# xxayt/MGSV

Hardware: AMD Instinct MI355X
Metric: video-music pairs/s fwd+bwd at B=64 (full training step); sub-objects: retrieval sim-matrix GB/s, eval forward pairs/s (higher is better)
Workload: dtype bf16; 1 GPU; BASELINE.json configs[2]: B=64/GPU, T_v=30, T_a=512, D=512, train mode (dropout on), f32 master weights + Adam, f32 gradient accumulation; global_batch=64, launch=tape

## Files before the change

include/made_hip.h:

```cpp
#ifndef MADE_HIP_H
#define MADE_HIP_H

#include <stdint.h>

#ifdef __cplusplus
extern "C" {
#endif

#define MADE_ABI_VERSION 8

enum MadeDtype { MADE_F32 = 0, MADE_BF16 = 1 };

enum MadeAct {
    MADE_ACT_NONE = 0,
    MADE_ACT_RELU = 1,
    MADE_ACT_GELU = 2,
    MADE_ACT_QUICKGELU = 3,
    MADE_ACT_SIGMOID = 4
};

enum MadeGate {
    MADE_GATE_NONE = 0,
    MADE_GATE_RELU_OUT = 1,
    MADE_GATE_GELU_Z = 2,
// ... 54 lines not shown
    int32_t use_a2;
    int32_t _pad;
} MadeLinearSeg;

typedef struct MadeLinearArgs {
    const void*  A;  int32_t a_dtype; int32_t w_dtype;
    int64_t      lda;
    const void*  A2; int64_t lda2; int64_t a2_row_mod;
    int32_t      a2_replace;
    int32_t      drop_col_div;
    const float* a_row_mask;
    const void*  W;  int64_t ldw;
    const float* bias;
    int64_t      M, N, K;
    int64_t      batch, a_z_stride, w_z_stride;
    int32_t      act; int32_t r_dtype;
    const void*  R;  int64_t ldr; int64_t r_row_mod;
    const float* out_row_mask;
    const float* tile_skip_mask;
    int32_t      nseg; int32_t split_k;
    float*       split_ws;
    MadeLinearSeg seg[4];
    const void*  G;  int32_t g_dtype; int32_t gate;
    int64_t      ldg; float gate_scale; int32_t z_dtype;
    void*        Zout; int64_t ldz;
    MadeDropout  drop; int64_t drop_ld;
    const int32_t* row_index; const int32_t* n_rows;
    const float* bias_row_scale; int64_t bias_z_stride;
} MadeLinearArgs;

int made_linear(const MadeLinearArgs* args, void* stream);

enum MadeLinearVariant {
    MADE_LINEAR_GENERAL_F32 = 0,
    MADE_LINEAR_GENERAL_F32IN = 1,
    MADE_LINEAR_GENERAL_BF16 = 2,
    MADE_LINEAR_TINY = 3,
    MADE_LINEAR_SKINNY = 4,
    MADE_LINEAR_GLDS3 = 5,
    MADE_LINEAR_GLDS64 = 6,
    MADE_LINEAR_GLDS128 = 7,
    MADE_LINEAR_BIG256 = 8,
    MADE_LINEAR_TINY16 = 9,
    MADE_LINEAR_BIG128 = 10,
    MADE_LINEAR_GLDS64_F32 = 11,
    MADE_LINEAR_GLDS128_F32 = 12
};
int made_linear_variant(const MadeLinearArgs* args);

typedef struct MadeDecStageArgs {
    const void*  Zin; int64_t ldz;
    const float* ln_g; const float* ln_b;
    const float* ln2_g; const float* ln2_b; void* x2_out; int64_t ldx2;
    const void*  add; int64_t add_row_mod;
    void*        x_out; int64_t ldx;
    const void*  W; int64_t ldw; const float* bias;
    const void*  R; int64_t ldr;
    void*        out; int64_t ldo;
    int32_t      out_dtype; int32_t act; int32_t res_from_x; float eps;
    int64_t      M, N, K;
    int32_t      zin_dtype; int32_t drop_col_div;
    void*        a_out; int64_t lda_out;
    MadeDropout  drop; int64_t drop_ld;
} MadeDecStageArgs;
int made_dec_stage(const MadeDecStageArgs* args, void* stream);

typedef struct MadeDecStageBwdArgs {
    const void* xa; const float* gamma_a; int64_t ldxa;
    const void* xb; const float* gamma_b; int64_t ldxb;
    const void* dy; int64_t lddy;
    const void* add; int64_t ldadd;
    void* dx_out; int64_t lddx;
    void* a_out; int64_t lda_out;
    float *dgamma_a, *dbeta_a, *dgamma_b, *dbeta_b;
    MadeDropout drop_a; int64_t drop_a_ld;
    const void* W; int64_t ldw;
    const void* G; int64_t ldg; float gate_scale; float eps;
    MadeDropout drop_o; int64_t drop_o_ld; int32_t drop_o_col_div; int32_t _pad;
    const void* R; int64_t ldr;
    void* out; int64_t ldo;
    int64_t M, N, K;
} MadeDecStageBwdArgs;
int made_dec_stage_bwd(const MadeDecStageBwdArgs* args, void* stream);

typedef struct MadeFinishArgs {
    const float* ws; int64_t split_k, M, N;
    const float* bias; int32_t act; int32_t r_dtype;
    const void*  R; int64_t ldr; int64_t r_row_mod;
    void* out; int32_t out_dtype; int32_t _pad0; int64_t ldo;
    const float* ln1_g; const float* ln1_b; void* ln1_out; int32_t ln1_dtype; int32_t _pad1; int64_t ln1_ld;
    const float* ln2_g; const float* ln2_b; void* ln2_out; int32_t ln2_dtype; int32_t _pad2; int64_t ln2_ld;
    float eps; int32_t _pad3;
} MadeFinishArgs;

int made_splitk_finish(const MadeFinishArgs* args, void* stream);

typedef struct MadeAttnArgs {
    const void* Q; const void* K; const void* V; void* O;
    int32_t dtype; int32_t hd;
    int64_t B, H, Lq, Lk;
    int64_t q_bs, ldq, k_bs, ldk, v_bs, ldv, o_bs, ldo;
    const float* key_mask; const float* q_mask;
    float scale; int32_t _pad;
    const float* q_skip_mask;
    float*      lse;
    MadeDropout drop;
    const int32_t* batch_order;
    uint32_t* keep_bits;
    int64_t ld_bits;
} MadeAttnArgs;

int made_attention(const MadeAttnArgs* args, void* stream);

typedef struct MadeWideAttnArgs {
    const void* Q; const void* K; const void* Kadd; const void* V; void* O;
    const float* key_mask;
    int32_t dtype; int32_t o_dtype;
    int64_t B, NQ1, NQ2, L, D;
    int64_t q_bs, q_s1, q_s2, k_bs, ldk, kadd_bs, ldkadd, v_bs, ldv, o_bs, o_s1, o_s2;
    float scale; int32_t _pad;
    int64_t n_split;
    float*  part_o;
    float*  part_ml;
    MadeDropout drop;
    float*  sum_out;
    float*  lse_out;
} MadeWideAttnArgs;

int made_attention_wide(const MadeWideAttnArgs* args, void* stream);

typedef struct MadeWideAttnBwdArgs {
    const void *Q, *dO, *O, *K, *V;
    const float* key_mask;
    const float *lse, *ssum;
    const float* extra;
    const void* dattc; int64_t ld_dattc; const float* vbias; int64_t hd;
    void *Pd, *dS; int64_t p_bs, ld_p;
    void* dQ; int64_t dq_bs, ld_dq;
    int64_t B, NQ, L, D;
    int64_t q_bs, ld_q, do_bs, ld_do, o_bs, ld_o, k_bs, ldk, v_bs, ldv;
    float scale; int32_t _pad;
    int64_t n_split; float* part_dq;
    MadeDropout drop;
} MadeWideAttnBwdArgs;
int made_attention_wide_bwd(const MadeWideAttnBwdArgs* args, void* stream);

#define MADE_WIDE_PLAN_HEAD 4
#define MADE_WIDE_PLAN_SAMPLE 4
#define MADE_WIDE_PLAN_SLOT 16
#define MADE_WIDE_PLAN_SLOT_BITS 8
MADE_HOST_DEVICE static inline int64_t made_wide_plan_words(int64_t B, int64_t n_slots) {
    return MADE_WIDE_PLAN_HEAD + MADE_WIDE_PLAN_SAMPLE * B + MADE_WIDE_PLAN_SLOT * n_slots;
}
MADE_HOST_DEVICE static inline int32_t made_wide_slice_count(const int32_t* tiles, int32_t stride, int32_t B, int32_t c, int32_t max_slices) {
    int32_t total = 0;
    for (int32_t b = 0; b < B; ++b) {
        const int32_t t = tiles[b * stride];
        const int32_t n = t > c ? (t + c - 1) / c : 1;
        if (n > max_slices) return -1;
        total += n;
    }
    return total;
}
MADE_HOST_DEVICE static inline int32_t made_wide_slice_cap(const int32_t* tiles, int32_t stride, int32_t B, int32_t n_slots, int32_t max_slices) {
    int32_t tmax = 1;
    for (int32_t b = 0; b < B; ++b) tmax = tiles[b * stride] > tmax ? tiles[b * stride] : tmax;
// ... 459 lines not shown
```

mgsv_amd/_lib.py:

```python
from __future__ import annotations

import ctypes as C
import os

_HERE = os.path.dirname(os.path.abspath(__file__))


def variant_env(name: str, default: str = "") -> str:
    if os.environ.get("MADE_DEBUG_VARIANTS", "0") in ("", "0"):
        return default
    return os.environ.get(name, default)


LIB_PATH = os.environ.get("MADE_LIB_PATH") or os.path.join(_HERE, "libmade_hip.so")
ABI_VERSION = 8

F32, BF16 = 0, 1
ACT_NONE, ACT_RELU, ACT_GELU, ACT_QUICKGELU, ACT_SIGMOID = 0, 1, 2, 3, 4
GATE_NONE, GATE_RELU_OUT, GATE_GELU_Z, GATE_QUICKGELU_Z, GATE_SIGMOID_OUT = 0, 1, 2, 3, 4

vp, i64, i32, f32 = C.c_void_p, C.c_int64, C.c_int32, C.c_float

WIDE_PLAN_HEAD, WIDE_PLAN_SAMPLE, WIDE_PLAN_SLOT, WIDE_PLAN_SLOT_BITS = 4, 4, 16, 8


def wide_plan_words(B: int, n_slots: int) -> int:
    return WIDE_PLAN_HEAD + WIDE_PLAN_SAMPLE * B + WIDE_PLAN_SLOT * n_slots


class MadeDropout(C.Structure):
    _fields_ = [("seed", C.c_uint64), ("site", C.c_uint32), ("p", f32), ("seed_device", vp)]


class MadeLinearSeg(C.Structure):
    _fields_ = [("col_begin", i64), ("out", vp), ("out_dtype", i32), ("transposed", i32), ("ldo", i64),
                ("rows_per_batch", i64), ("out_batch_stride", i64), ("out_z_stride", i64),
                ("use_a2", i32), ("_pad", i32)]


class MadeLinearArgs(C.Structure):
    _fields_ = [("A", vp), ("a_dtype", i32), ("w_dtype", i32), ("lda", i64),
                ("A2", vp), ("lda2", i64), ("a2_row_mod", i64),
                ("a2_replace", i32), ("drop_col_div", i32),
                ("a_row_mask", vp),
                ("W", vp), ("ldw", i64),
                ("bias", vp),
                ("M", i64), ("N", i64), ("K", i64),
                ("batch", i64), ("a_z_stride", i64), ("w_z_stride", i64),
                ("act", i32), ("r_dtype", i32),
                ("R", vp), ("ldr", i64), ("r_row_mod", i64),
                ("out_row_mask", vp),
                ("tile_skip_mask", vp),
                ("nseg", i32), ("split_k", i32),
                ("split_ws", vp),
                ("seg", MadeLinearSeg * 4),
                ("G", vp), ("g_dtype", i32), ("gate", i32), ("ldg", i64), ("gate_scale", f32), ("z_dtype", i32),
                ("Zout", vp), ("ldz", i64), ("drop", MadeDropout), ("drop_ld", i64), ("row_index", vp), ("n_rows", vp),
                ("bias_row_scale", vp), ("bias_z_stride", i64)]


class MadeFinishArgs(C.Structure):
    _fields_ = [("ws", vp), ("split_k", i64), ("M", i64), ("N", i64),
                ("bias", vp), ("act", i32), ("r_dtype", i32),
                ("R", vp), ("ldr", i64), ("r_row_mod", i64),
                ("out", vp), ("out_dtype", i32), ("_pad0", i32), ("ldo", i64),
                ("ln1_g", vp), ("ln1_b", vp), ("ln1_out", vp), ("ln1_dtype", i32), ("_pad1", i32), ("ln1_ld", i64),
                ("ln2_g", vp), ("ln2_b", vp), ("ln2_out", vp), ("ln2_dtype", i32), ("_pad2", i32), ("ln2_ld", i64),
                ("eps", f32), ("_pad3", i32)]


class MadeDecStageArgs(C.Structure):
    _fields_ = [("Zin", vp), ("ldz", i64), ("ln_g", vp), ("ln_b", vp),
                ("ln2_g", vp), ("ln2_b", vp), ("x2_out", vp), ("ldx2", i64),
                ("add", vp), ("add_row_mod", i64), ("x_out", vp), ("ldx", i64),
                ("W", vp), ("ldw", i64), ("bias", vp), ("R", vp), ("ldr", i64), ("out", vp), ("ldo", i64),
                ("out_dtype", i32), ("act", i32), ("res_from_x", i32), ("eps", f32),
                ("M", i64), ("N", i64), ("K", i64),
                ("zin_dtype", i32), ("drop_col_div", i32), ("a_out", vp), ("lda_out", i64), ("drop", MadeDropout), ("drop_ld", i64)]


class MadeDecStageBwdArgs(C.Structure):
    _fields_ = [("xa", vp), ("gamma_a", vp), ("ldxa", i64), ("xb", vp), ("gamma_b", vp), ("ldxb", i64), ("dy", vp), ("lddy", i64),
                ("add", vp), ("ldadd", i64), ("dx_out", vp), ("lddx", i64), ("a_out", vp), ("lda_out", i64),
                ("dgamma_a", vp), ("dbeta_a", vp), ("dgamma_b", vp), ("dbeta_b", vp), ("drop_a", MadeDropout), ("drop_a_ld", i64),
                ("W", vp), ("ldw", i64), ("G", vp), ("ldg", i64), ("gate_scale", f32), ("eps", f32),
                ("drop_o", MadeDropout), ("drop_o_ld", i64), ("drop_o_col_div", i32), ("_pad", i32),
                ("R", vp), ("ldr", i64), ("out", vp), ("ldo", i64), ("M", i64), ("N", i64), ("K", i64)]


class MadeAttnArgs(C.Structure):
    _fields_ = [("Q", vp), ("K", vp), ("V", vp), ("O", vp),
                ("dtype", i32), ("hd", i32),
                ("B", i64), ("H", i64), ("Lq", i64), ("Lk", i64),
                ("q_bs", i64), ("ldq", i64), ("k_bs", i64), ("ldk", i64),
                ("v_bs", i64), ("ldv", i64), ("o_bs", i64), ("ldo", i64),
                ("key_mask", vp), ("q_mask", vp),
                ("scale", f32), ("_pad", i32),
                ("q_skip_mask", vp),
                ("lse", vp), ("drop", MadeDropout), ("batch_order", vp), ("keep_bits", vp), ("ld_bits", i64)]


class MadeAttnBwdArgs(C.Structure):
    _fields_ = [("Q", vp), ("K", vp), ("V", vp), ("O", vp), ("dO", vp), ("dQ", vp), ("dK", vp), ("dV", vp),
                ("lse", vp), ("delta", vp), ("dtype", i32), ("hd", i32),
                ("B", i64), ("H", i64), ("Lq", i64), ("Lk", i64),
                ("q_bs", i64), ("ldq", i64), ("k_bs", i64), ("ldk", i64), ("v_bs", i64), ("ldv", i64), ("o_bs", i64), ("ldo", i64),
                ("do_bs", i64), ("lddo", i64), ("dq_bs", i64), ("lddq", i64), ("dk_bs", i64), ("lddk", i64), ("dv_bs", i64), ("lddv", i64),
                ("key_mask", vp), ("q_skip_mask", vp), ("scale", f32), ("_pad", i32), ("drop", MadeDropout),
                ("batch_order", vp), ("keep_bits", vp), ("ld_bits", i64)]


class MadeXpoolFusedArgs(C.Structure):
    _fields_ = [("Q", vp), ("ldq", i64), ("K", vp), ("U", vp), ("k_bs", i64), ("ldk", i64), ("u_bs", i64), ("ldu", i64),
                ("key_mask", vp), ("ln2_g", vp), ("ln2_b", vp), ("Wl", vp), ("ldw", i64), ("bl", vp), ("ln3_g", vp), ("ln3_b", vp),
                ("vn", vp), ("ldvn", i64), ("sims", vp), ("ld_sims", i64),
                ("Nv", i64), ("Nm", i64), ("S", i64), ("D", i64), ("scale", f32), ("eps", f32), ("ws", vp), ("prepare_ws", i32), ("_pad", i32)]


class MadeXpoolAttnArgs(C.Structure):
    _fields_ = [("Q", vp), ("ldq", i64), ("K", vp), ("U", vp), ("k_bs", i64), ("ldk", i64), ("u_bs", i64), ("ldu", i64),
                ("key_mask", vp), ("out", vp), ("ldo", i64), ("Nv", i64), ("Nm", i64), ("S", i64), ("D", i64),
                ("scale", f32), ("eps", f32), ("normalize", i32), ("_pad", i32), ("ws", vp)]


class MadeXpoolSimsArgs(C.Structure):
    _fields_ = [("Q", vp), ("ldq", i64), ("K", vp), ("UU", vp), ("k_bs", i64), ("ldk", i64), ("u_bs", i64), ("ldu", i64),
                ("key_mask", vp), ("av", vp), ("bv", vp), ("ln3_g", vp), ("ln3_b", vp), ("vn", vp), ("ldvn", i64),
                ("sims", vp), ("ld_sims", i64), ("Nv", i64), ("Nm", i64), ("S", i64), ("D", i64),
                ("scale", f32), ("eps", f32), ("ws", vp), ("prepare_ws", i32), ("_pad", i32)]


class MadeXpoolPairsArgs(C.Structure):
    _fields_ = [("Q", vp), ("ldq", i64), ("K", vp), ("UU", vp), ("k_bs", i64), ("ldk", i64), ("u_bs", i64), ("ldu", i64),
                ("key_mask", vp), ("av", vp), ("bv", vp), ("ln3_g", vp), ("ln3_b", vp), ("vn", vp), ("ldvn", i64),
                ("start", vp), ("video", vp), ("score", vp), ("Nv", i64), ("U", i64), ("P", i64), ("S", i64), ("D", i64),
                ("max_count", i64), ("scale", f32), ("eps", f32)]


class MadeXpoolInbatchArgs(C.Structure):
    _fields_ = [("Q", vp), ("ldq", i64), ("K", vp), ("U", vp), ("k_bs", i64), ("ldk", i64), ("u_bs", i64), ("ldu", i64),
                ("key_mask", vp), ("out", vp), ("out_dtype", i32), ("_pad", i32), ("o_bs", i64), ("ldo", i64),
                ("Nv", i64), ("Nm", i64), ("S", i64), ("D", i64), ("scale", f32), ("_pad2", i32), ("ws", vp)]


class MadeWideAttnArgs(C.Structure):
    _fields_ = [("Q", vp), ("K", vp), ("Kadd", vp), ("V", vp), ("O", vp), ("key_mask", vp),
                ("dtype", i32), ("o_dtype", i32),
                ("B", i64), ("NQ1", i64), ("NQ2", i64), ("L", i64), ("D", i64),
                ("q_bs", i64), ("q_s1", i64), ("q_s2", i64), ("k_bs", i64), ("ldk", i64), ("kadd_bs", i64), ("ldkadd", i64),
                ("v_bs", i64), ("ldv", i64), ("o_bs", i64), ("o_s1", i64), ("o_s2", i64),
                ("scale", f32), ("_pad", i32),
                ("n_split", i64), ("part_o", vp), ("part_ml", vp), ("drop", MadeDropout), ("sum_out", vp),
                ("lse_out", vp)]


class MadeWideAttnBwdArgs(C.Structure):
    _fields_ = ([(k, vp) for k in ("Q", "dO", "O", "K", "V", "key_mask", "lse", "ssum", "extra", "dattc")] + [("ld_dattc", i64), ("vbias", vp), ("hd", i64),
                ("Pd", vp), ("dS", vp), ("p_bs", i64), ("ld_p", i64), ("dQ", vp), ("dq_bs", i64), ("ld_dq", i64)] +
                [(k, i64) for k in ("B", "NQ", "L", "D", "q_bs", "ld_q", "do_bs", "ld_do", "o_bs", "ld_o", "k_bs", "ldk", "v_bs", "ldv")] +
                [("scale", f32), ("_pad", i32), ("n_split", i64), ("part_dq", vp), ("drop", MadeDropout)])


class MadeGemmTNArgs(C.Structure):
    _fields_ = [("A", vp), ("B", vp), ("C", vp), ("ab_dtype", i32), ("c_dtype", i32),
                ("M", i64), ("N", i64), ("K", i64), ("lda", i64), ("ldb", i64), ("ldc", i64),
                ("batch1", i64), ("batch2", i64),
                ("a_zs1", i64), ("a_zs2", i64), ("b_zs1", i64), ("b_zs2", i64), ("c_zs1", i64), ("c_zs2", i64),
                ("row_mask", vp), ("mask_zs1", i64), ("mask_zs2", i64),
                ("alpha", f32), ("accumulate", i32), ("split_m", i64),
                ("colsum", vp), ("colsum_zs1", i64), ("colsum_zs2", i64), ("row_group_valid", vp),
                ("row_index", vp), ("n_rows", vp)]


class MadeGemmTNProblem(C.Structure):
    _fields_ = [("A", vp), ("B", vp), ("C", vp), ("colsum", vp), ("N", i64), ("K", i64), ("lda", i64), ("ldb", i64), ("ldc", i64)]


class MadeGemmTNGroup(C.Structure):
    _fields_ = [("n_problems", i32), ("alpha", f32), ("M", i64), ("split_m", i64), ("row_index", vp), ("n_rows", vp),
                ("p", MadeGemmTNProblem * 8), ("tile_end", i32 * 8), ("tile_size", i32), ("_pad", i32),
                ("workspace", vp), ("workspace_bytes", i64)]


class MadeAdamGroup(C.Structure):
    _fields_ = [("begin", i64), ("end", i64), ("lr", f32), ("max_norm", f32)]


class MadeAdamDeviceState(C.Structure):
    _fields_ = [("step", i64), ("lr", f32 * 4), ("bc1", f32), ("bc2_sqrt", f32)]


class MadeRepackDesc(C.Structure):
    _fields_ = [("src", vp), ("w", vp), ("wt", vp), ("rows", i64), ("cols", i64), ("wt_ld", i64), ("tile_begin", i64),
                ("dtype", i32), ("_pad", i32)]


class MadeFrameDesc(C.Structure):
    _fields_ = [("offset", i64), ("coef", i64), ("H", i32), ("W", i32), ("kh", i32), ("kv", i32)]


class MadeResampleDesc(C.Structure):
    _fields_ = [("offset", i64), ("n", i64), ("taps", i64), ("o", i32), ("m", i32), ("width", i32), ("_pad", i32)]


class MadeAudioSegDesc(C.Structure):
    _fields_ = [("first", i64), ("count", i64)]


GATHER_MAX_ARRAYS = 8
GATHER_F32, GATHER_BF16, GATHER_U8 = 0, 1, 2


class MadeGatherArray(C.Structure):
    _fields_ = [("src", vp), ("row", vp), ("dst", vp), ("rows", i64), ("row_elems", i64), ("kind", i32), ("_pad", i32)]


class MadeGatherBatchArgs(C.Structure):
    _fields_ = [("a", MadeGatherArray * GATHER_MAX_ARRAYS), ("index", vp), ("n_samples", i64), ("B", i64), ("n_arrays", i32), ("_pad", i32)]


SIGNATURES = {
    "made_abi_version": (C.c_int, []),
    "made_set_f32_products": (C.c_int, [C.c_int]),
    "made_get_f32_products": (C.c_int, []),
    "made_last_error": (C.c_char_p, []),
    "made_device_info": (C.c_int, [C.c_char_p, C.c_int, C.POINTER(C.c_int), C.POINTER(C.c_int)]),
    "made_tape_begin": (C.c_int, []),
    "made_tape_end": (C.c_int, [C.POINTER(C.c_uint64)]),
    "made_tape_replay": (C.c_int, [C.c_uint64]),
    "made_tape_free": (C.c_int, [C.c_uint64]),
    "made_tape_interleave": (C.c_int, [C.c_uint64, i32]),
    "made_tape_count": (C.c_int, [C.c_uint64, C.POINTER(i64), C.POINTER(i64), C.POINTER(i64)]),
    "made_tape_replay_range": (C.c_int, [C.c_uint64, i64, i64]),
    "made_tape_op": (C.c_int, [C.c_uint64, i64, C.POINTER(i32), C.POINTER(C.c_uint64), C.POINTER(C.c_uint64), C.POINTER(C.c_uint32)]),
    "made_stream_wait": (C.c_int, [vp, vp]),
    "made_tape_event": (C.c_int, [i32, i32, vp]),
    "made_tape_callback": (C.c_int, [C.CFUNCTYPE(C.c_int, vp), vp]),
    "made_memset_async": (C.c_int, [vp, i32, i64, vp]),
    "made_copy_async": (C.c_int, [vp, vp, i64, vp]),
    "made_store_words": (C.c_int, [vp, vp, i32, vp]),
    "made_linear": (C.c_int, [C.POINTER(MadeLinearArgs), vp]),
    "made_splitk_finish": (C.c_int, [C.POINTER(MadeFinishArgs), vp]),
    "made_dec_stage": (C.c_int, [C.POINTER(MadeDecStageArgs), vp]),
    "made_dec_stage_bwd": (C.c_int, [C.POINTER(MadeDecStageBwdArgs), vp]),
    "made_attention": (C.c_int, [C.POINTER(MadeAttnArgs), vp]),
    "made_attention_wide": (C.c_int, [C.POINTER(MadeWideAttnArgs), vp]),
    "made_attention_wide_bwd": (C.c_int, [C.POINTER(MadeWideAttnBwdArgs), vp]),
    "made_wide_slice_plan": (C.c_int, [vp, i64, i64, i32, i32, vp, vp, i64, vp]),
    "made_attention_wide_planned": (C.c_int, [C.POINTER(MadeWideAttnArgs), vp, i32, vp]),
    "made_attention_wide_bwd_planned": (C.c_int, [C.POINTER(MadeWideAttnBwdArgs), vp, i32, vp]),
    "made_layernorm": (C.c_int, [vp, i32, i64, i64, i64, vp, vp, vp, i32, i64, i64, i64, f32, vp, vp]),
    "made_layernorm_add": (C.c_int, [vp, i32, i64, vp, vp, vp, i32, i64, vp, i32, i64, vp, i64, i64, i64, f32, vp, vp]),
    "made_cast_mask_rows": (C.c_int, [vp, i64, vp, vp, i32, i64, i64, i64, vp]),
    "made_pack_music_records": (C.c_int, [vp, i32, i64, vp, i64, vp, i64, vp, i32, i64, i64, i64, i64, i64, vp]),
    "made_masked_mean": (C.c_int, [vp, i32, i64, i64, vp, vp, i64, i64, i64, vp]),
    "made_l2norm_rows": (C.c_int, [vp, i32, i64, vp, vp, i32, i64, i64, i64, f32, vp]),
    "made_sine_pe": (C.c_int, [vp, vp, vp, i32, i64, i64, i64, vp]),
    "made_masked_softmax": (C.c_int, [vp, i64, vp, i64, vp, i32, i64, i64, i64, i64, i64, f32, vp]),
    "made_xpool_tail": (C.c_int, [vp, i32, i64, vp, vp, vp, i64, vp, vp, i64, i64, i64, i64, f32, vp]),
    "made_clip_loss": (C.c_int, [vp, i64, i64, vp, f32, i32, vp, vp, vp]),
    "made_hungarian_match": (C.c_int, [vp, vp, vp, i64, i64, i64, i64, i32, f32, f32, f32, vp, i32, vp, vp, vp, vp, vp]),
    "made_attention_bwd": (C.c_int, [C.POINTER(MadeAttnBwdArgs), vp]),
    "made_layernorm_bwd": (C.c_int, [vp, i32, i64, i64, i64, vp, vp, i32, i64, vp, i32, i64, vp, i32, i64, vp, i64,
                                     C.POINTER(MadeDropout), i64, vp, vp, i64, i64, f32, vp, vp]),
    "made_layernorm_bwd2": (C.c_int, [vp, vp, i64, vp, vp, i64, vp, i64, vp, i64, vp, i64, vp, i64, C.POINTER(MadeDropout), i64, i32,
                                      vp, vp, vp, vp, i64, i64, f32, vp]),
    "made_pool_bwd": (C.c_int, [vp, vp, vp, vp, i32, i64, i64, vp, i32, i64, i64, vp, i32, i64, i64, i64, i64, i64, f32, vp]),
    "made_l2norm_bwd": (C.c_int, [vp, i32, i64, vp, i64, i64, vp, i64, i32, vp, i32, i64, i64, i64, f32, vp]),
    "made_clip_loss_bwd": (C.c_int, [vp, i64, i64, vp, f32, vp, vp, vp, vp, i32, vp, vp, vp]),
    "made_xpool_tail_bwd": (C.c_int, [vp, i32, i64, vp, vp, vp, i64, vp, i64, vp, i32, i64, vp, C.POINTER(MadeDropout),
                                      vp, vp, vp, i64, vp, i64, f32, i64, i64, i64, f32, vp]),
    "made_softmax_bwd": (C.c_int, [vp, i64, vp, i64, vp, i64, vp, f32, C.POINTER(MadeDropout), vp, vp, vp, i32, i64, i64,
                                   i64, i64, i64, i64, i64, vp]),
    "made_head_bias": (C.c_int, [vp, i32, i64, vp, vp, i64, i64, i64, vp]),
    "made_head_bias_bwd": (C.c_int, [vp, i32, i64, vp, vp, vp, vp, i64, i64, i64, vp]),
    "made_add3": (C.c_int, [vp, i32, vp, i32, vp, i32, vp, i32, i64, i64, vp]),
    "made_colsum": (C.c_int, [vp, i32, i64, i64, i64, vp, vp]),
    "made_posbn_relu_fwd": (C.c_int, [vp, i32, i64, vp, vp, vp, vp, C.c_float, C.c_float, i32, vp, vp, vp, i32, i64, i64, i64, i64, vp]),
    "made_posbn_relu_bwd": (C.c_int, [vp, i32, i64, vp, i32, i64, vp, i32, i64, vp, vp, vp, i32, vp, i32, i64, vp, vp, i64, i64, i64, vp]),
    "made_set_criterion_bwd": (C.c_int, [vp, vp, vp, vp, vp, vp, vp, vp, vp, i64, i64, i64, i64, i64, i32, f32, vp, vp,
                                         vp, vp, i64, i32, vp, vp, vp]),
    "made_adam_step": (C.c_int, [vp, vp, vp, vp, i64, C.POINTER(MadeAdamGroup), i32, f32, f32, f32, i64, f32, vp, vp]),
    "made_adam_step_device": (C.c_int, [vp, vp, vp, vp, i64, C.POINTER(MadeAdamGroup), i32, f32, f32, f32, vp, i32, f32, vp, vp]),
    "made_repack": (C.c_int, [vp, i32, i64, vp]),
    "made_row_groups": (C.c_int, [vp, i64, vp, vp]),
    "made_row_index": (C.c_int, [vp, i64, vp, vp, vp]),
    "made_linear_variant": (C.c_int, [C.POINTER(MadeLinearArgs)]),
    "made_row_affine": (C.c_int, [vp, i32, i64, vp, vp, i64, i32, vp, i32, i64, i64, i64, vp]),
    "made_gate_rows": (C.c_int, [vp, i32, i64, vp, i32, i64, i32, f32, vp, i64, i64, vp, i32, i64, vp, i64, i64, vp]),
    "made_xpool_fused": (C.c_int, [C.POINTER(MadeXpoolFusedArgs), vp]),
    "made_xpool_attention": (C.c_int, [C.POINTER(MadeXpoolAttnArgs), vp]),
    "made_xpool_sims": (C.c_int, [C.POINTER(MadeXpoolSimsArgs), vp]),
    "made_xpool_sims_ws_bytes": (C.c_int64, [i64, i64, i64]),
    "made_xpool_sims_pairs": (C.c_int, [C.POINTER(MadeXpoolPairsArgs), vp]),
    "made_xpool_inbatch": (C.c_int, [C.POINTER(MadeXpoolInbatchArgs), vp]),
    "made_xpool_inbatch_ws_bytes": (C.c_int64, [i64, i64]),
    "made_batch_order": (C.c_int, [vp, i64, i64, vp, vp]),
    "made_recall_ranks": (C.c_int, [vp, i64, vp, vp, i64, i64, i64, vp, vp, vp]),
    "made_span_iou": (C.c_int, [vp, vp, vp, vp, i64, i64, i32, f32, vp, vp, vp]),
    "made_gemm_tn": (C.c_int, [C.POINTER(MadeGemmTNArgs), vp]),
    "made_gemm_tn_grouped": (C.c_int, [C.POINTER(MadeGemmTNGroup), vp]),
    "made_gemm_tn_grouped_workspace": (i64, [C.POINTER(MadeGemmTNGroup)]),
    "made_concat_cols": (C.c_int, [vp, i64, vp, i64, vp, i64, vp]),
    "made_pooled_cosine": (C.c_int, [vp, i64, vp, i32, vp, i64, i64, i64, i64, i64, vp]),
    "made_scale_exp": (C.c_int, [vp, vp, vp, i64, vp]),
    "made_span_convert": (C.c_int, [vp, vp, i64, i32, vp]),
    "made_span_pairwise": (C.c_int, [vp, vp, vp, vp, vp, vp, i64, i64, vp]),
    "made_span_iou_se": (C.c_int, [vp, vp, vp, i64, f32, i32, i32, vp, vp]),
    "made_set_criterion": (C.c_int, [vp, vp, vp, vp, vp, vp, vp, vp, vp, i64, i64, i64, i64, i64, i32, f32, vp, vp, vp, vp]),
    "made_topk_groups_ws_bytes": (C.c_int64, [i64, i64, i64]),
    "made_topk_groups": (C.c_int, [vp, i64, vp, i64, i64, i64, i64, vp, vp, vp, i64, vp]),
    "made_eligibility": (C.c_int, [vp, vp, vp, vp, vp, vp, vp, vp, vp, vp, i64, i64, i64, vp, i64, vp, vp]),
    "made_topk_groups_masked": (C.c_int, [vp, i64, vp, vp, i64, i64, i64, i64, i64, vp, vp, vp, i64, vp]),
    "made_gather_pairs": (C.c_int, [vp, vp, i64, i64, i64, vp, i64, vp, i64, vp, i64, vp, i64, vp, i64, vp, i64, i64, i64, i64, i32,
                                    vp, i64, vp, i64, vp, vp, vp, vp, vp]),
    "made_gather_rows": (C.c_int, [vp, i64, vp, i64, i64, vp, i32, vp]),
    "made_group_topw": (C.c_int, [vp, i64, vp, vp, vp, vp, i64, i64, i64, i64, i64, i64, vp, vp, vp]),
    "made_group_topw_masked": (C.c_int, [vp, i64, vp, i64, vp, vp, vp, vp, i64, i64, i64, i64, i64, i64, vp, vp, vp]),
    "made_topk_merge": (C.c_int, [vp, vp, i64, vp, vp, i64, i64, i64, i64, i64, vp, vp, vp]),
    "made_topk_candidates": (C.c_int, [vp, vp, i64, i64, vp, i64, i64, i64, i64, vp, vp, vp]),
    "made_mmr_select": (C.c_int, [vp, vp, vp, i64, i64, i64, i64, i64, f32, f32, vp, vp, vp]),
    "made_cosine_join": (C.c_int, [vp, i64, i64, vp, i64, i64, i64, i64, f32, vp, vp, vp, i64, vp, vp]),
    "made_cosine_topk_ws_bytes": (C.c_int64, [i64, i64, i64, i32]),
    "made_cosine_topk": (C.c_int, [vp, i64, vp, vp, i64, i64, vp, i64, i32, vp, vp, vp, i64, vp]),
    "made_cosine_topk_ex_ws_bytes": (C.c_int64, [i64, i64, i64, i32, i32]),
    "made_cosine_topk_ex": (C.c_int, [vp, i64, vp, vp, i64, i64, vp, vp, i64, i64, i32, i32, vp, vp, vp, i64, vp]),
    "made_merge_moments": (C.c_int, [vp, vp, vp, vp, vp, i64, i64, i64, i64, i32, f32, f32, i64, vp, vp, vp, vp, vp]),
# ... 62 lines not shown
```

mgsv_amd/csrc/decoder.hip:

```cpp
#include "common.h"
#include <type_traits>

namespace {

constexpr int DS_BM = 16, DS_BN = 16, DS_THREADS = 256, DS_RPW = 4, DS_CT_LD = DS_BN + 4;

__device__ __forceinline__ float ds_act(float x, int act) {
    return act == MADE_ACT_RELU ? fmaxf(x, 0.f) : x;
}

template <int NV, bool ZB16, bool TRAIN>
__global__ __launch_bounds__(DS_THREADS) void dec_stage_kernel(const MadeDecStageArgs a) {
    constexpr int K = 64 * NV;
    constexpr int LDA = K * 2 + 16;
    constexpr int STEPS = NV / 2;
    __shared__ __attribute__((aligned(16))) unsigned char dlds[DS_BM * LDA];
    __shared__ __attribute__((aligned(16))) float Ct[4 * DS_BM * DS_CT_LD];
    const int tid = threadIdx.x;
    const int lane = tid & 63, wave = __builtin_amdgcn_readfirstlane(tid >> 6);
    const int r16 = lane & 15, kq = lane >> 4;
    const int M = (int)a.M, N = (int)a.N;
    const int n0 = blockIdx.x * DS_BN, m0 = blockIdx.y * DS_BM;

    const int kw = wave * (K / 4) + kq * 8;
    int gn = n0 + r16; gn = gn < N ? gn : N - 1;
    const bf16_t* pw = (const bf16_t*)a.W + (int64_t)gn * a.ldw + kw;
    bf16x8 fw[STEPS];
#pragma unroll
    for (int s = 0; s < STEPS; ++s) fw[s] = *(const bf16x8*)(pw + s * 32);

    constexpr int RPW = DS_RPW;
    const int c0 = NV * lane;
    const bool has_ln = a.ln_g != nullptr, has_ln2 = a.ln2_g != nullptr && a.x2_out != nullptr;
    float v[RPW][NV];
#pragma unroll
    for (int i = 0; i < RPW; ++i) {
        int gm = m0 + wave * RPW + i; gm = gm < M ? gm : M - 1;
        if constexpr (ZB16) {
            const bf16_t* zp = (const bf16_t*)a.Zin + (int64_t)gm * a.ldz + c0;
            if constexpr (NV == 8) {
                const bf16x8 t = *(const bf16x8*)zp;
#pragma unroll
                for (int u = 0; u < 8; ++u) v[i][u] = (float)t[u];
            } else {
                const bf16x4 t = *(const bf16x4*)zp;
#pragma unroll
                for (int u = 0; u < 4; ++u) v[i][u] = (float)t[u];
            }
        } else {
            const float* zp = (const float*)a.Zin + (int64_t)gm * a.ldz + c0;
#pragma unroll
            for (int j = 0; j < NV; j += 4) {
                const f32x4 t = *(const f32x4*)(zp + j);
                v[i][j] = t[0]; v[i][j + 1] = t[1]; v[i][j + 2] = t[2]; v[i][j + 3] = t[3];
            }
        }
    }
    float g1[NV], b1[NV], g2[NV], b2[NV];
#pragma unroll
    for (int j = 0; j < NV; ++j) { g1[j] = 1.f; b1[j] = 0.f; g2[j] = 1.f; b2[j] = 0.f; }
    if (has_ln) {
#pragma unroll
        for (int j = 0; j < NV; j += 4) {
            const f32x4 g = *(const f32x4*)(a.ln_g + c0 + j), b = *(const f32x4*)(a.ln_b + c0 + j);
#pragma unroll
            for (int u = 0; u < 4; ++u) { g1[j + u] = g[u]; b1[j + u] = b[u]; }
        }
    }
    if (has_ln2) {
#pragma unroll
        for (int j = 0; j < NV; j += 4) {
            const f32x4 g = *(const f32x4*)(a.ln2_g + c0 + j), b = *(const f32x4*)(a.ln2_b + c0 + j);
#pragma unroll
            for (int u = 0; u < 4; ++u) { g2[j + u] = g[u]; b2[j + u] = b[u]; }
        }
    }
    const int add_mod = (int)a.add_row_mod;
    const bool add_same = a.add != nullptr && add_mod == 1;
    float ad[RPW][NV];
    if (a.add) {
#pragma unroll
        for (int i = 0; i < RPW; ++i) {
            if (add_same && i > 0) {
#pragma unroll
                for (int u = 0; u < NV; ++u) ad[i][u] = ad[0][u];
                continue;
            }
            int gm = m0 + wave * RPW + i; gm = gm < M ? gm : M - 1;
            const bf16_t* ap = (const bf16_t*)a.add + (int64_t)(add_same ? 0 : gm % add_mod) * K + c0;
            if constexpr (NV == 8) {
                const bf16x8 t = *(const bf16x8*)ap;
#pragma unroll
                for (int u = 0; u < 8; ++u) ad[i][u] = (float)t[u];
            } else {
                const bf16x4 t = *(const bf16x4*)ap;
#pragma unroll
                for (int u = 0; u < 4; ++u) ad[i][u] = (float)t[u];
            }
        }
    }
    float y2[RPW][NV];
#pragma unroll
    for (int i = 0; i < RPW; ++i) {
        const int rl = wave * RPW + i;
        if (has_ln) {
            if constexpr (ZB16) {
                float s = 0.f, q = 0.f;
#pragma unroll
                for (int j = 0; j < NV; ++j) { s += v[i][j]; q += v[i][j] * v[i][j]; }
                s = wave_sum(s); q = wave_sum(q);
                const float mean = s * (1.f / K);
                const float rstd = rsqrtf(fmaxf(q * (1.f / K) - mean * mean, 0.f) + a.eps);
#pragma unroll
                for (int j = 0; j < NV; ++j) v[i][j] = (v[i][j] - mean) * rstd * g1[j] + b1[j];
            } else {
                float s = 0.f;
#pragma unroll
                for (int j = 0; j < NV; ++j) s += v[i][j];
                const float mean = wave_sum(s) * (1.f / K);
                float q = 0.f;
#pragma unroll
                for (int j = 0; j < NV; ++j) { v[i][j] -= mean; q += v[i][j] * v[i][j]; }
                const float rstd = rsqrtf(wave_sum(q) * (1.f / K) + a.eps);
#pragma unroll
                for (int j = 0; j < NV; ++j) v[i][j] = v[i][j] * rstd * g1[j] + b1[j];
            }
        }
        if (has_ln2) {
            float s = 0.f;
#pragma unroll
            for (int j = 0; j < NV; ++j) s += v[i][j];
            const float mean = wave_sum(s) * (1.f / K);
            float q = 0.f;
#pragma unroll
            for (int j = 0; j < NV; ++j) { const float d = v[i][j] - mean; q += d * d; }
            const float rstd = rsqrtf(wave_sum(q) * (1.f / K) + a.eps);
#pragma unroll
            for (int j = 0; j < NV; ++j) y2[i][j] = (v[i][j] - mean) * rstd * g2[j] + b2[j];
        }
        if constexpr (NV == 8) {
            bf16x8 t;
#pragma unroll
            for (int u = 0; u < 8; ++u) t[u] = a.add ? (bf16_t)((float)(bf16_t)v[i][u] + ad[i][u]) : (bf16_t)v[i][u];
            *(bf16x8*)(dlds + rl * LDA + c0 * 2) = t;
        } else {
            bf16x4 t;
#pragma unroll
            for (int u = 0; u < 4; ++u) t[u] = a.add ? (bf16_t)((float)(bf16_t)v[i][u] + ad[i][u]) : (bf16_t)v[i][u];
            *(bf16x4*)(dlds + rl * LDA + c0 * 2) = t;
        }
    }
    const int cc = tid & 1, row = (tid >> 1) & 15;
    const int n = n0 + cc * 8;
    int nvalid = N - n; nvalid = nvalid > 8 ? 8 : nvalid;
    const int ml = m0 + row;
    const int mlc = ml < M ? ml : M - 1;
    float bv[8];
#pragma unroll
    for (int j = 0; j < 8; ++j) bv[j] = 0.f;
    if (a.bias) {
#pragma unroll
        for (int j = 0; j < 8; ++j) { const int nj = n + j < N ? n + j : N - 1; bv[j] = a.bias[nj]; }
    }
    const bool r_vec = a.R && nvalid == 8 && (a.ldr % 8 == 0) && (((uintptr_t)a.R & 15) == 0);
    bf16x8 rpre;
    if (r_vec) rpre = *(const bf16x8*)((const bf16_t*)a.R + (int64_t)mlc * a.ldr + n);

#pragma unroll
    for (int i = 0; i < RPW; ++i) {
        const int gm = m0 + wave * RPW + i;
        const bool writer = (gm < M) && (gm % (int)gridDim.x == (int)blockIdx.x);
        if (!writer) continue;
        if (a.x_out) {
            bf16_t* xp = (bf16_t*)a.x_out + (int64_t)gm * a.ldx + c0;
            if constexpr (NV == 8) { bf16x8 t; for (int u = 0; u < 8; ++u) t[u] = (bf16_t)v[i][u]; *(bf16x8*)xp = t; }
            else { bf16x4 t; for (int u = 0; u < 4; ++u) t[u] = (bf16_t)v[i][u]; *(bf16x4*)xp = t; }
        }
        if (TRAIN && a.a_out) {
            bf16_t* ap = (bf16_t*)a.a_out + (int64_t)gm * a.lda_out + c0;
            if constexpr (NV == 8) { bf16x8 t; for (int u = 0; u < 8; ++u) t[u] = a.add ? (bf16_t)((float)(bf16_t)v[i][u] + ad[i][u]) : (bf16_t)v[i][u]; *(bf16x8*)ap = t; }
            else { bf16x4 t; for (int u = 0; u < 4; ++u) t[u] = a.add ? (bf16_t)((float)(bf16_t)v[i][u] + ad[i][u]) : (bf16_t)v[i][u]; *(bf16x4*)ap = t; }
        }
        if (has_ln2) {
            bf16_t* yp = (bf16_t*)a.x2_out + (int64_t)gm * a.ldx2 + c0;
            if constexpr (NV == 8) { bf16x8 t; for (int u = 0; u < 8; ++u) t[u] = (bf16_t)y2[i][u]; *(bf16x8*)yp = t; }
            else { bf16x4 t; for (int u = 0; u < 4; ++u) t[u] = (bf16_t)y2[i][u]; *(bf16x4*)yp = t; }
        }
    }
    __syncthreads();

    f32x4 acc;
    acc[0] = acc[1] = acc[2] = acc[3] = 0.f;
#pragma unroll
    for (int s = 0; s < STEPS; ++s) {
        const bf16x8 fa = *(const bf16x8*)(dlds + r16 * LDA + (kw + s * 32) * 2);
        acc = __builtin_amdgcn_mfma_f32_16x16x32_bf16(fa, fw[s], acc, 0, 0, 0);
    }

    float xres[8];
#pragma unroll
    for (int j = 0; j < 8; ++j) xres[j] = 0.f;
    if (a.res_from_x && n + 8 <= K) {
        const bf16x8 t = *(const bf16x8*)(dlds + row * LDA + n * 2);
#pragma unroll
        for (int j = 0; j < 8; ++j) xres[j] = (float)t[j];
    }
    {
        float* mine = Ct + wave * (DS_BM * DS_CT_LD);
#pragma unroll
        for (int e = 0; e < 4; ++e) mine[(kq * 4 + e) * DS_CT_LD + r16] = acc[e];
    }
    __syncthreads();
    if (tid >= 32 || nvalid <= 0 || ml >= M) return;
    float v8[8];
#pragma unroll
    for (int j = 0; j < 8; ++j) v8[j] = 0.f;
    float rv[8];
#pragma unroll
    for (int j = 0; j < 8; ++j) rv[j] = xres[j];
    const bool vec = nvalid == 8;
    if (a.R) {
        if (r_vec) {
#pragma unroll
            for (int j = 0; j < 8; ++j) rv[j] = (float)rpre[j];
        } else {
            for (int j = 0; j < nvalid; ++j) rv[j] = (float)((const bf16_t*)a.R)[(int64_t)ml * a.ldr + n + j];
        }
    }
#pragma unroll
    for (int w = 0; w < 4; ++w) {
        const float* cp = Ct + w * (DS_BM * DS_CT_LD) + row * DS_CT_LD + cc * 8;
        const f32x4 q0 = *(const f32x4*)cp, q1 = *(const f32x4*)(cp + 4);
        v8[0] += q0[0]; v8[1] += q0[1]; v8[2] += q0[2]; v8[3] += q0[3];
        v8[4] += q1[0]; v8[5] += q1[1]; v8[6] += q1[2]; v8[7] += q1[3];
    }
    const int act = a.act;
#pragma unroll
    for (int j = 0; j < 8; ++j) v8[j] = ds_act(v8[j] + bv[j], act);
    if constexpr (TRAIN) {
        if (a.drop.p > 0.f) {
            const uint32_t thr = made_drop_threshold(a.drop.p);
            const float sc = 1.f / (1.f - a.drop.p);
            const uint64_t seed = made_drop_seed(a.drop);
            const uint64_t rb = (uint64_t)ml * (uint64_t)a.drop_ld;
            const int div = a.drop_col_div > 1 ? a.drop_col_div : 1;
            if (div == 1) {
                const uint32_t kb = made_keep_bits<8>(seed, a.drop.site, thr, rb + (uint64_t)n);
#pragma unroll
                for (int j = 0; j < 8; ++j) v8[j] = ((kb >> j) & 1u) ? v8[j] * sc : 0.f;
            } else {
#pragma unroll
                for (int j = 0; j < 8; ++j)
                    v8[j] = (made_rng_mix(seed, a.drop.site, rb + (uint64_t)((n + j) / div)) >> 8) >= thr ? v8[j] * sc : 0.f;
            }
        }
    }
#pragma unroll
    for (int j = 0; j < 8; ++j) v8[j] += rv[j];
    if (a.out_dtype == MADE_F32) {
        float* op = (float*)a.out + (int64_t)ml * a.ldo + n;
        if (vec && (a.ldo % 4 == 0) && (((uintptr_t)a.out & 15) == 0)) {
            f32x4 o0, o1;
            o0[0] = v8[0]; o0[1] = v8[1]; o0[2] = v8[2]; o0[3] = v8[3]; o1[0] = v8[4]; o1[1] = v8[5]; o1[2] = v8[6]; o1[3] = v8[7];
            *(f32x4*)op = o0; *(f32x4*)(op + 4) = o1;
        } else {
            for (int j = 0; j < nvalid; ++j) op[j] = v8[j];
        }
    } else {
        bf16_t* op = (bf16_t*)a.out + (int64_t)ml * a.ldo + n;
        if (vec && (a.ldo % 8 == 0) && (((uintptr_t)a.out & 15) == 0)) {
            bf16x8 o;
#pragma unroll
            for (int j = 0; j < 8; ++j) o[j] = (bf16_t)v8[j];
            *(bf16x8*)op = o;
        } else {
            for (int j = 0; j < nvalid; ++j) op[j] = (bf16_t)v8[j];
        }
    }
}

template <int NV>
__device__ __forceinline__ void dsb_ln_bwd_row(float (&xv)[NV], float (&gy)[NV], const float (&gm)[NV], float eps, float (&dg)[NV], float (&db)[NV], float (&o)[NV]) {
    constexpr int K = 64 * NV;
    float sx = 0.f, sxx = 0.f, sg = 0.f, sgx = 0.f;
#pragma unroll
    for (int j = 0; j < NV; ++j) {
        const float g = gy[j] * gm[j];
        sx += xv[j]; sxx += xv[j] * xv[j]; sg += g; sgx += g * xv[j];
    }
    sx = wave_sum(sx); sxx = wave_sum(sxx); sg = wave_sum(sg); sgx = wave_sum(sgx);
    const float mean = sx * (1.f / K);
    const float var = fmaxf(sxx * (1.f / K) - mean * mean, 0.f);
    const float rstd = 1.0f / sqrtf(var + eps);
    const float s1 = sg * (1.f / K);
    const float s2 = rstd * (sgx - mean * sg) * (1.f / K);
#pragma unroll
    for (int j = 0; j < NV; ++j) {
        const float xh = (xv[j] - mean) * rstd;
        dg[j] += gy[j] * xh; db[j] += gy[j];
        o[j] = rstd * (gy[j] * gm[j] - s1 - xh * s2);
    }
}

template <int NV>
__device__ __forceinline__ void dsb_load_row(const void* p, int64_t off, float (&v)[NV]) {
    if constexpr (NV == 8) {
        const bf16x8 t = *(const bf16x8*)((const bf16_t*)p + off);
#pragma unroll
        for (int u = 0; u < 8; ++u) v[u] = (float)t[u];
    } else {
        const bf16x4 t = *(const bf16x4*)((const bf16_t*)p + off);
#pragma unroll
        for (int u = 0; u < 4; ++u) v[u] = (float)t[u];
    }
}
template <int NV>
__device__ __forceinline__ void dsb_store_row(void* p, int64_t off, const float (&v)[NV]) {
    if constexpr (NV == 8) { bf16x8 t; for (int u = 0; u < 8; ++u) t[u] = (bf16_t)v[u]; *(bf16x8*)((bf16_t*)p + off) = t; }
    else { bf16x4 t; for (int u = 0; u < 4; ++u) t[u] = (bf16_t)v[u]; *(bf16x4*)((bf16_t*)p + off) = t; }
}

template <int NV, int MODE>
__global__ __launch_bounds__(DS_THREADS) void dec_stage_bwd_kernel(const MadeDecStageBwdArgs a) {
    constexpr bool TWO = MODE == 2, ADD1 = MODE == 1;
    constexpr int K = 64 * NV;
    constexpr int LDA = K * 2 + 16;
    constexpr int STEPS = NV / 2;
    __shared__ __attribute__((aligned(16))) unsigned char dlds[DS_BM * LDA];
    __shared__ __attribute__((aligned(16))) float Ct[4 * DS_BM * DS_CT_LD];
    __shared__ float pgrad[4 * (TWO ? 4 : 2) * K];
    constexpr int PV = TWO ? 4 : 2;
    const int tid = threadIdx.x;
    const int lane = tid & 63, wave = __builtin_amdgcn_readfirstlane(tid >> 6);
    const int r16 = lane & 15, kq = lane >> 4;
    const int M = (int)a.M, N = (int)a.N;
    const int n0 = blockIdx.x * DS_BN, m0 = blockIdx.y * DS_BM;
    constexpr bool two = TWO;

    const int kw = wave * (K / 4) + kq * 8;
    int gn = n0 + r16; gn = gn < N ? gn : N - 1;
    const bf16_t* pw = (const bf16_t*)a.W + (int64_t)gn * a.ldw + kw;
    bf16x8 fw[STEPS];
#pragma unroll
    for (int s = 0; s < STEPS; ++s) fw[s] = *(const bf16x8*)(pw + s * 32);
    const int cc = tid & 1, row = (tid >> 1) & 15;
    const int n = n0 + cc * 8;
    int nvalid = N - n; nvalid = nvalid > 8 ? 8 : nvalid;
    const int ml = m0 + row;
    const int mlc = ml < M ? ml : M - 1;
    const bool e_vec = nvalid == 8;
    bf16x8 rpre, gpre;
    const bool r_vec = a.R && e_vec && (a.ldr % 8 == 0) && (((uintptr_t)a.R & 15) == 0);
    const bool g_vec = a.G && e_vec && (a.ldg % 8 == 0) && (((uintptr_t)a.G & 15) == 0);
    if (r_vec) rpre = *(const bf16x8*)((const bf16_t*)a.R + (int64_t)mlc * a.ldr + n);
    if (g_vec) gpre = *(const bf16x8*)((const bf16_t*)a.G + (int64_t)mlc * a.ldg + n);

    const int c0 = NV * lane;
    float gma[NV], gmb[NV];
#pragma unroll
    for (int j = 0; j < NV; j += 4) {
        const f32x4 g = *(const f32x4*)(a.gamma_a + c0 + j);
        gma[j] = g[0]; gma[j + 1] = g[1]; gma[j + 2] = g[2]; gma[j + 3] = g[3];
        if (two) { const f32x4 h = *(const f32x4*)(a.gamma_b + c0 + j); gmb[j] = h[0]; gmb[j + 1] = h[1]; gmb[j + 2] = h[2]; gmb[j + 3] = h[3]; }
        else { gmb[j] = gmb[j + 1] = gmb[j + 2] = gmb[j + 3] = 1.f; }
    }
    float dga[NV], dba[NV], dgb[NV], dbb[NV];
#pragma unroll
    for (int j = 0; j < NV; ++j) { dga[j] = 0.f; dba[j] = 0.f; dgb[j] = 0.f; dbb[j] = 0.f; }
    const uint32_t thr = made_drop_threshold(a.drop_a.p);
    const uint64_t seed_a = a.drop_a.p > 0.f ? made_drop_seed(a.drop_a) : 0;
    const float sc_a = a.drop_a.p > 0.f ? 1.f / (1.f - a.drop_a.p) : 1.f;
    constexpr int RPW = DS_RPW;
    typedef typename std::conditional<NV == 8, bf16x8, bf16x4>::type raw_t;
    raw_t rxa[RPW], rdy[RPW], rxb[TWO ? RPW : 1], rad[(TWO || ADD1) ? RPW : 1];
#pragma unroll
    for (int i = 0; i < RPW; ++i) {
        int gm = m0 + wave * RPW + i; gm = gm < M ? gm : M - 1;
        rxa[i] = *(const raw_t*)((const bf16_t*)a.xa + (int64_t)gm * a.ldxa + c0);
        rdy[i] = *(const raw_t*)((const bf16_t*)a.dy + (int64_t)gm * a.lddy + c0);
    }
    if constexpr (TWO) {
#pragma unroll
        for (int i = 0; i < RPW; ++i) {
            int gm = m0 + wave * RPW + i; gm = gm < M ? gm : M - 1;
            rxb[i] = *(const raw_t*)((const bf16_t*)a.xb + (int64_t)gm * a.ldxb + c0);
            rad[i] = *(const raw_t*)((const bf16_t*)(a.add ? a.add : a.xb) + (int64_t)gm * (a.add ? a.ldadd : a.ldxb) + c0);
        }
    }
    if constexpr (ADD1) {
#pragma unroll
        for (int i = 0; i < RPW; ++i) {
            int gm = m0 + wave * RPW + i; gm = gm < M ? gm : M - 1;
            rad[i] = *(const raw_t*)((const bf16_t*)a.add + (int64_t)gm * a.ldadd + c0);
        }
    }
#pragma unroll
    for (int i = 0; i < RPW; ++i) {
        const int rl = wave * RPW + i;
        int gm = m0 + rl; gm = gm < M ? gm : M - 1;
        const bool real = m0 + rl < M;
        float xa[NV], gy[NV], o[NV];
#pragma unroll
        for (int j = 0; j < NV; ++j) { xa[j] = (float)rxa[i][j]; gy[j] = (float)rdy[i][j]; }
        if constexpr (ADD1) {
#pragma unroll
            for (int j = 0; j < NV; ++j) gy[j] += (float)rad[i][j];
        }
        if constexpr (TWO) {
            float xb[NV], ad[NV], g[NV];
#pragma unroll
            for (int j = 0; j < NV; ++j) { xb[j] = (float)rxb[i][j]; ad[j] = a.add ? (float)rad[i][j] : 0.f; }
            float tg[NV], tb[NV];
#pragma unroll
            for (int j = 0; j < NV; ++j) { tg[j] = 0.f; tb[j] = 0.f; }
            dsb_ln_bwd_row<NV>(xb, gy, gmb, a.eps, tg, tb, g);
#pragma unroll
            for (int j = 0; j < NV; ++j) { if (real) { dgb[j] += tg[j]; dbb[j] += tb[j]; } gy[j] = g[j] + ad[j]; }
        }
        float tg[NV], tb[NV];
#pragma unroll
        for (int j = 0; j < NV; ++j) { tg[j] = 0.f; tb[j] = 0.f; }
        dsb_ln_bwd_row<NV>(xa, gy, gma, a.eps, tg, tb, o);
#pragma unroll
        for (int j = 0; j < NV; ++j) { if (real) { dga[j] += tg[j]; dba[j] += tb[j]; } }
        float od[NV];
        const uint64_t dbase = (uint64_t)gm * (uint64_t)a.drop_a_ld + (uint64_t)c0;
        const uint32_t kb = a.drop_a.p > 0.f ? made_keep_bits<NV>(seed_a, a.drop_a.site, thr, dbase) : 0xFFu;
#pragma unroll
        for (int j = 0; j < NV; ++j) od[j] = ((kb >> j) & 1u) ? o[j] * sc_a : 0.f;
        dsb_store_row<NV>(dlds, (int64_t)rl * (LDA / 2) + c0, od);
        const bool writer = real && ((m0 + rl) % (int)gridDim.x == (int)blockIdx.x);
        if (writer) {
            if (a.dx_out) dsb_store_row<NV>(a.dx_out, (int64_t)gm * a.lddx + c0, o);
            if (a.a_out) dsb_store_row<NV>(a.a_out, (int64_t)gm * a.lda_out + c0, od);
        }
    }
    if (blockIdx.x == 0) {
        float* mine = pgrad + wave * PV * K;
#pragma unroll
        for (int j = 0; j < NV; ++j) {
            mine[c0 + j] = dga[j]; mine[K + c0 + j] = dba[j];
            if constexpr (TWO) { mine[2 * K + c0 + j] = dgb[j]; mine[3 * K + c0 + j] = dbb[j]; }
        }
    }
    __syncthreads();

    f32x4 acc;
    acc[0] = acc[1] = acc[2] = acc[3] = 0.f;
#pragma unroll
    for (int s = 0; s < STEPS; ++s) {
        const bf16x8 fa = *(const bf16x8*)(dlds + r16 * LDA + (kw + s * 32) * 2);
        acc = __builtin_amdgcn_mfma_f32_16x16x32_bf16(fa, fw[s], acc, 0, 0, 0);
    }
    {
        float* mine = Ct + wave * (DS_BM * DS_CT_LD);
#pragma unroll
        for (int e = 0; e < 4; ++e) mine[(kq * 4 + e) * DS_CT_LD + r16] = acc[e];
    }
    if (blockIdx.x == 0) {
        for (int c = tid; c < PV * K; c += DS_THREADS) {
            float t = 0.f;
#pragma unroll
            for (int w = 0; w < 4; ++w) t += pgrad[w * PV * K + c];
            float* dst = c < K ? a.dgamma_a : (c < 2 * K ? a.dbeta_a : (c < 3 * K ? a.dgamma_b : a.dbeta_b));
            if (dst) unsafeAtomicAdd(dst + (c % K), t);
        }
    }
    __syncthreads();
    if (tid >= 32 || nvalid <= 0 || ml >= M) return;

    float v8[8];
#pragma unroll
    for (int j = 0; j < 8; ++j) v8[j] = 0.f;
#pragma unroll
    for (int w = 0; w < 4; ++w) {
        const float* cp = Ct + w * (DS_BM * DS_CT_LD) + row * DS_CT_LD + cc * 8;
        const f32x4 q0 = *(const f32x4*)cp, q1 = *(const f32x4*)(cp + 4);
        v8[0] += q0[0]; v8[1] += q0[1]; v8[2] += q0[2]; v8[3] += q0[3];
        v8[4] += q1[0]; v8[5] += q1[1]; v8[6] += q1[2]; v8[7] += q1[3];
    }
    if (a.G) {
        float g8[8];
        if (g_vec) {
#pragma unroll
            for (int j = 0; j < 8; ++j) g8[j] = (float)gpre[j];
        } else {
            for (int j = 0; j < 8; ++j) g8[j] = j < nvalid ? (float)((const bf16_t*)a.G)[(int64_t)ml * a.ldg + n + j] : 0.f;
        }
#pragma unroll
        for (int j = 0; j < 8; ++j) v8[j] = g8[j] != 0.f ? v8[j] * a.gate_scale : 0.f;
    }
    if (a.drop_o.p > 0.f) {
        const uint32_t thr_o = made_drop_threshold(a.drop_o.p);
        const float sc = 1.f / (1.f - a.drop_o.p);
        const uint64_t seed_o = made_drop_seed(a.drop_o);
        const uint64_t rb = (uint64_t)ml * (uint64_t)a.drop_o_ld;
        const int div = a.drop_o_col_div > 1 ? a.drop_o_col_div : 1;
#pragma unroll
        for (int j = 0; j < 8; ++j)
            v8[j] = (made_rng_mix(seed_o, a.drop_o.site, rb + (uint64_t)((n + j) / div)) >> 8) >= thr_o ? v8[j] * sc : 0.f;
    }
    if (a.R) {
        if (r_vec) {
#pragma unroll
            for (int j = 0; j < 8; ++j) v8[j] += (float)rpre[j];
        } else {
            for (int j = 0; j < nvalid; ++j) v8[j] += (float)((const bf16_t*)a.R)[(int64_t)ml * a.ldr + n + j];
        }
    }
    bf16_t* op = (bf16_t*)a.out + (int64_t)ml * a.ldo + n;
    if (e_vec && (a.ldo % 8 == 0) && (((uintptr_t)a.out & 15) == 0)) {
        bf16x8 o8;
#pragma unroll
        for (int j = 0; j < 8; ++j) o8[j] = (bf16_t)v8[j];
        *(bf16x8*)op = o8;
    } else {
        for (int j = 0; j < nvalid; ++j) op[j] = (bf16_t)v8[j];
    }
}

}

extern "C" int made_dec_stage_bwd(const MadeDecStageBwdArgs* args, void* stream) {
    MADE_REQUIRE(args != nullptr, "made_dec_stage_bwd: null args");
    const MadeDecStageBwdArgs& a = *args;
    MADE_REQUIRE(a.xa && a.gamma_a && a.dy && a.W && a.out, "made_dec_stage_bwd: null xa, gamma_a, dy, W or out");
    MADE_REQUIRE((a.xb == nullptr) == (a.gamma_b == nullptr), "made_dec_stage_bwd: xb and gamma_b come together");
    MADE_REQUIRE(a.M > 0 && a.N > 0, "made_dec_stage_bwd: bad dims M=%lld N=%lld", (long long)a.M, (long long)a.N);
    MADE_UNSUPPORTED(a.K == 256 || a.K == 512, "made_dec_stage_bwd: K=%lld (the row width of the LayerNorm) must be 256 or 512", (long long)a.K);
    MADE_UNSUPPORTED(a.ldxa % 8 == 0 && a.lddy % 8 == 0 && a.ldxb % 8 == 0 && a.ldadd % 8 == 0 && a.lddx % 8 == 0 && a.lda_out % 8 == 0 && a.ldw % 8 == 0 &&
                     ((uintptr_t)a.xa % 16) == 0 && ((uintptr_t)a.dy % 16) == 0 && ((uintptr_t)a.xb % 16) == 0 && ((uintptr_t)a.add % 16) == 0 &&
                     ((uintptr_t)a.dx_out % 16) == 0 && ((uintptr_t)a.a_out % 16) == 0 && ((uintptr_t)a.W % 16) == 0,
                     "made_dec_stage_bwd: rows must be 16-byte aligned");
    MADE_REQUIRE(a.drop_a.p >= 0.f && a.drop_a.p < 1.f && a.drop_o.p >= 0.f && a.drop_o.p < 1.f, "made_dec_stage_bwd: dropout p out of [0,1)");
    const dim3 grid((unsigned)((a.N + DS_BN - 1) / DS_BN), (unsigned)((a.M + DS_BM - 1) / DS_BM)), block(DS_THREADS);
    hipStream_t st = (hipStream_t)stream;
    if (a.K == 512) {
        if (a.xb) hipLaunchKernelGGL((dec_stage_bwd_kernel<8, 2>), grid, block, 0, st, a);
        else if (a.add) hipLaunchKernelGGL((dec_stage_bwd_kernel<8, 1>), grid, block, 0, st, a);
        else hipLaunchKernelGGL((dec_stage_bwd_kernel<8, 0>), grid, block, 0, st, a);
    } else {
        if (a.xb) hipLaunchKernelGGL((dec_stage_bwd_kernel<4, 2>), grid, block, 0, st, a);
        else if (a.add) hipLaunchKernelGGL((dec_stage_bwd_kernel<4, 1>), grid, block, 0, st, a);
        else hipLaunchKernelGGL((dec_stage_bwd_kernel<4, 0>), grid, block, 0, st, a);
    }
    return made_check_launch("made_dec_stage_bwd");
}

extern "C" int made_dec_stage(const MadeDecStageArgs* args, void* stream) {
    MADE_REQUIRE(args != nullptr, "made_dec_stage: null args");
    const MadeDecStageArgs& a = *args;
    MADE_REQUIRE(a.Zin && a.W && a.out, "made_dec_stage: null Zin, W or out");
    MADE_REQUIRE(a.M > 0 && a.N > 0, "made_dec_stage: bad dims M=%lld N=%lld", (long long)a.M, (long long)a.N);
    MADE_UNSUPPORTED(a.K == 256 || a.K == 512, "made_dec_stage: K=%lld (the row width of the LayerNorm) must be 256 or 512", (long long)a.K);
    MADE_UNSUPPORTED(a.ldz % 4 == 0 && ((uintptr_t)a.Zin % 16) == 0, "made_dec_stage: Zin rows must be 16-byte aligned");
    MADE_UNSUPPORTED(a.ldw % 8 == 0 && ((uintptr_t)a.W % 16) == 0, "made_dec_stage: W rows must be 16-byte aligned");
    MADE_REQUIRE((a.ln_g == nullptr) == (a.ln_b == nullptr) && (a.ln2_g == nullptr) == (a.ln2_b == nullptr), "made_dec_stage: gamma and beta come together");
    MADE_REQUIRE(a.out_dtype == MADE_F32 || a.out_dtype == MADE_BF16, "made_dec_stage: bad out_dtype %d", a.out_dtype);
    MADE_UNSUPPORTED(a.act == MADE_ACT_NONE || a.act == MADE_ACT_RELU, "made_dec_stage: act=%d (ReLU or none)", a.act);
    if (a.x_out) MADE_UNSUPPORTED(a.ldx % 8 == 0 && ((uintptr_t)a.x_out % 16) == 0, "made_dec_stage: x_out rows must be 16-byte aligned");
    if (a.x2_out) MADE_UNSUPPORTED(a.ldx2 % 8 == 0 && ((uintptr_t)a.x2_out % 16) == 0, "made_dec_stage: x2_out rows must be 16-byte aligned");
    if (a.add) MADE_REQUIRE(a.add_row_mod >= 1 && ((uintptr_t)a.add % 16) == 0, "made_dec_stage: add needs add_row_mod >= 1 and 16-byte alignment");
    if (a.res_from_x) MADE_REQUIRE(a.N == a.K && a.add == nullptr && a.R == nullptr, "made_dec_stage: res_from_x needs N == K, no add, no R");
    const bool train = a.drop.p > 0.f || a.a_out != nullptr;
    MADE_REQUIRE(a.zin_dtype == MADE_F32 || a.zin_dtype == MADE_BF16, "made_dec_stage: bad zin_dtype %d", a.zin_dtype);
    MADE_REQUIRE(a.drop.p >= 0.f && a.drop.p < 1.f, "made_dec_stage: dropout p out of [0,1)");
    if (a.a_out) MADE_UNSUPPORTED(a.lda_out % 8 == 0 && ((uintptr_t)a.a_out % 16) == 0, "made_dec_stage: a_out rows must be 16-byte aligned");
    if (a.zin_dtype == MADE_BF16) MADE_UNSUPPORTED(a.ldz % 8 == 0, "made_dec_stage: bf16 Zin rows must be 16-byte aligned");
    MADE_UNSUPPORTED((a.zin_dtype == MADE_BF16) == train || !train, "made_dec_stage: dropout / a_out need bf16 Zin rows");
    const bool tr = a.zin_dtype == MADE_BF16;
    const dim3 grid((unsigned)((a.N + DS_BN - 1) / DS_BN), (unsigned)((a.M + DS_BM - 1) / DS_BM)), block(DS_THREADS);
    hipStream_t st = (hipStream_t)stream;
    if (a.K == 512) {
        if (tr) hipLaunchKernelGGL((dec_stage_kernel<8, true, true>), grid, block, 0, st, a);
        else hipLaunchKernelGGL((dec_stage_kernel<8, false, false>), grid, block, 0, st, a);
    } else {
        if (tr) hipLaunchKernelGGL((dec_stage_kernel<4, true, true>), grid, block, 0, st, a);
        else hipLaunchKernelGGL((dec_stage_kernel<4, false, false>), grid, block, 0, st, a);
    }
    return made_check_launch("made_dec_stage");
}
```

mgsv_amd/ops.py:

```python
from __future__ import annotations

import ctypes as C
import math
from dataclasses import dataclass
from typing import NamedTuple, Optional, Sequence, Tuple

import torch

from . import _lib, tape as _tape
from ._lib import (ACT_GELU, ACT_NONE, ACT_QUICKGELU, ACT_RELU, ACT_SIGMOID, BF16, F32,
                   MadeAttnArgs, MadeDecStageArgs, MadeFinishArgs, MadeLinearArgs, MadeLinearSeg, MadeWideAttnArgs, check, lib)

Tensor = torch.Tensor


def dt_of(t: Tensor) -> int:
    if t.dtype == torch.float32:
        return F32
    if t.dtype == torch.bfloat16:
        return BF16
    raise TypeError(f"unsupported dtype {t.dtype}")


def torch_dtype(code: int):
    return torch.float32 if code == F32 else torch.bfloat16


def _p(t: Optional[Tensor]):
    if t is None:
        return None
    if not t.is_cuda:
        raise _lib.MadeError("libmade_hip ops need GPU tensors (no CPU fallback)")
    if _tape._recording is not None:
        _tape._recording._keep.append(t)
    return t.data_ptr()


def _stream():
    return torch.cuda.current_stream().cuda_stream


def _f32(t: Optional[Tensor], name: str) -> Optional[Tensor]:
    if t is not None and (t.dtype != torch.float32 or not t.is_contiguous()):
        raise TypeError(f"{name} must be a contiguous float32 tensor")
    return t


def set_drop(d, drop) -> None:
    seed, site, p = drop
    if isinstance(seed, Tensor):
        assert seed.dtype == torch.int64 and seed.numel() == 1 and seed.is_cuda
        d.seed, d.seed_device = 0, seed.data_ptr()
    else:
        d.seed, d.seed_device = int(seed) & 0xFFFFFFFFFFFFFFFF, None
    d.site, d.p = int(site) & 0xFFFFFFFF, float(p)


def round_up(x: int, m: int) -> int:
    return (x + m - 1) // m * m


class KernelTimer:

    def __init__(self):
        self.records = []

    def __enter__(self):
        global _timer
        self._prev, _timer = _timer, self
        return self

    def __exit__(self, *exc):
        global _timer
        _timer = self._prev

    def summary(self):
        torch.cuda.synchronize()
        out = {}
        frac_cache = {}
        for kind, s, e, flops, nbytes, desc in self.records:
            d = out.setdefault(kind, dict(launches=0, ms=0.0, flops=0.0, bytes=0.0, flops_nominal=0.0))
            d["launches"] += 1
            d["ms"] += s.elapsed_time(e)
            frac = 1.0
            if isinstance(desc, tuple) and desc[0] == "rows":
                frac = min(1.0, (math.ceil(int(desc[1].item()) / 128) * 128) / max(desc[2], 1))
            elif isinstance(desc, tuple) and desc[0] == "attn":
                key = ("attn", desc[1].data_ptr() if desc[1] is not None else 0, desc[2].data_ptr() if desc[2] is not None else 0)
                if key not in frac_cache:
                    fk = (desc[1] != 0).float().mean(dim=1) if desc[1] is not None else 1.0
                    fq = (desc[2] != 0).float().mean(dim=1) if desc[2] is not None else 1.0
                    f = fk * fq
                    frac_cache[key] = float(f.mean().item()) if isinstance(f, torch.Tensor) else 1.0
                frac = frac_cache[key]
# ... 121 lines not shown
                           f"G={None if G is None else str(G.dtype)[6:]} Z={None if Zout is None else str(Zout.dtype)[6:]} "
                           f"drop={0 if drop is None else drop[2]}/{drop_col_div} rows={int(rows is not None)} orm={int(out_row_mask is not None)} "
                           f"arm={int(a_row_mask is not None)} out={str(segs[0].out.dtype)[6:]} rpb={segs[0].rows_per_batch} tr={int(any(s_.transposed for s_ in segs))}"))
    _timed(kind, flops, nbytes, lambda: check(lib().made_linear(C.byref(a), _stream()), "made_linear"),
           ("rows", rows[1], M) if rows is not None else ((desc, tile_skip_mask, 128) if tile_skip_mask is not None else desc))
    return segs[0].out


def row_index(mask: Tensor, out=None):
    m = mask.reshape(-1)
    M = m.numel()
    if out is not None:
        idx, n = out
        assert idx.dtype == torch.int32 and idx.numel() >= M and n.dtype == torch.int32
    else:
        idx = torch.empty(M, device=m.device, dtype=torch.int32)
        n = torch.empty(1, device=m.device, dtype=torch.int32)
    check(lib().made_row_index(_p(_f32(m, "mask")), M, _p(idx), _p(n), _stream()), "made_row_index")
    return idx, n


def batch_order(mask: Tensor, out: Optional[Tensor] = None) -> Tensor:
    assert mask.dim() == 2
    B, T = mask.shape
    if out is None:
        out = torch.empty(B, device=mask.device, dtype=torch.int32)
    assert out.dtype == torch.int32 and out.numel() == B
    check(lib().made_batch_order(_p(_f32(mask.contiguous(), "mask")), B, T, _p(out), _stream()), "made_batch_order")
    return out


def linear_splitk(A: Tensor, W: Tensor, bias: Optional[Tensor], ws: Tensor, split_k: int, *, A2: Optional[Tensor] = None,
                  a2_row_mod: int = 0, act: int = ACT_NONE, R: Optional[Tensor] = None, r_row_mod: int = 0,
                  out: Optional[Tensor] = None, ln1=None, ln1_out: Optional[Tensor] = None, ln2=None,
                  ln2_out: Optional[Tensor] = None, eps: float = 1e-5) -> None:
    assert A.dim() == 2 and W.dim() == 2 and A.stride(1) == 1 and W.stride(1) == 1
    M, K = A.shape
    N = W.shape[0]
    assert ws.dtype == torch.float32 and ws.is_contiguous() and ws.numel() >= split_k * M * N
    a = MadeLinearArgs()
    a.A, a.a_dtype, a.w_dtype, a.lda = _p(A), dt_of(A), dt_of(W), A.stride(0)
    use_a2 = A2 is not None
    if use_a2:
        a.A2, a.lda2, a.a2_row_mod = _p(A2), A2.stride(0), a2_row_mod
    a.W, a.ldw = _p(W), W.stride(0)
    a.M, a.N, a.K = M, N, K
    a.batch = 1
    a.nseg, a.split_k, a.split_ws = 1, max(split_k, 2), _p(ws)
    sg = a.seg[0]
    sg.col_begin, sg.out, sg.out_dtype, sg.ldo, sg.use_a2 = 0, _p(ws), F32, N, 1 if use_a2 else 0
    esz = 4 if a.w_dtype == F32 else 2
    _timed("linear_splitk_f32" if a.w_dtype == F32 else "linear_kernel<bf16,bf16>", 2.0 * M * N * K, M * K * esz + N * K * esz + M * N * 4 * a.split_k,
           lambda: check(lib().made_linear(C.byref(a), _stream()), "made_linear(split_k)"), f"M={M} N={N} K={K} split={a.split_k}")
    splitk_finish(ws, a.split_k, M, N, bias, act=act, R=R, r_row_mod=r_row_mod, out=out, ln1=ln1, ln1_out=ln1_out, ln2=ln2, ln2_out=ln2_out,
                  eps=eps)


def splitk_finish(ws: Tensor, split_k: int, M: int, N: int, bias: Optional[Tensor], *, act: int = ACT_NONE, R: Optional[Tensor] = None,
                  r_row_mod: int = 0, out: Optional[Tensor] = None, ln1=None, ln1_out: Optional[Tensor] = None, ln2=None,
                  ln2_out: Optional[Tensor] = None, eps: float = 1e-5) -> None:
    assert ws.dtype == torch.float32 and ws.is_contiguous() and ws.numel() >= split_k * M * N
    f = MadeFinishArgs()
    f.ws, f.split_k, f.M, f.N = _p(ws), split_k, M, N
    f.bias, f.act = _p(_f32(bias, "bias")), act
    if R is not None:
        assert R.dim() == 2 and R.stride(1) == 1
        f.R, f.r_dtype, f.ldr, f.r_row_mod = _p(R), dt_of(R), R.stride(0), r_row_mod
    if out is not None:
        f.out, f.out_dtype, f.ldo = _p(out), dt_of(out), out.stride(0)
    if ln1 is not None:
        f.ln1_g, f.ln1_b = _p(_f32(ln1[0], "ln1.g")), _p(_f32(ln1[1], "ln1.b"))
        if ln1_out is not None:
            f.ln1_out, f.ln1_dtype, f.ln1_ld = _p(ln1_out), dt_of(ln1_out), ln1_out.stride(0)
    if ln2 is not None:
        f.ln2_g, f.ln2_b = _p(_f32(ln2[0], "ln2.g")), _p(_f32(ln2[1], "ln2.b"))
        f.ln2_out, f.ln2_dtype, f.ln2_ld = _p(ln2_out), dt_of(ln2_out), ln2_out.stride(0)
    f.eps = eps
    check(lib().made_splitk_finish(C.byref(f), _stream()), "made_splitk_finish")


def dec_stage(Zin: Tensor, W: Tensor, bias: Optional[Tensor], out: Tensor, *, ln=None, ln2=None, x2_out: Optional[Tensor] = None,
              add: Optional[Tensor] = None, x_out: Optional[Tensor] = None, R: Optional[Tensor] = None, res_from_x: bool = False,
              act: int = ACT_NONE, eps: float = 1e-5, a_out: Optional[Tensor] = None, drop=None, drop_ld: Optional[int] = None,
              drop_col_div: int = 1) -> Tensor:
    assert Zin.dim() == 2 and W.dim() == 2 and out.dim() == 2 and W.dtype == torch.bfloat16
    assert Zin.stride(1) == 1 and W.stride(1) == 1 and out.stride(1) == 1
    M, K = Zin.shape
    N = W.shape[0]
    assert W.shape[1] == K and tuple(out.shape) == (M, N)
    a = MadeDecStageArgs()
    a.Zin, a.ldz, a.zin_dtype = _p(Zin), Zin.stride(0), dt_of(Zin)
    if ln is not None:
        a.ln_g, a.ln_b = _p(_f32(ln[0], "ln.g")), _p(_f32(ln[1], "ln.b"))
    if ln2 is not None:
        assert x2_out is not None and x2_out.dtype == torch.bfloat16 and x2_out.stride(1) == 1
        a.ln2_g, a.ln2_b, a.x2_out, a.ldx2 = _p(_f32(ln2[0], "ln2.g")), _p(_f32(ln2[1], "ln2.b")), _p(x2_out), x2_out.stride(0)
    if add is not None:
        assert add.dim() == 2 and add.dtype == torch.bfloat16 and add.is_contiguous() and add.shape[1] == K
        a.add, a.add_row_mod = _p(add), add.shape[0]
    if x_out is not None:
        assert x_out.dtype == torch.bfloat16 and x_out.stride(1) == 1 and tuple(x_out.shape) == (M, K)
        a.x_out, a.ldx = _p(x_out), x_out.stride(0)
    if a_out is not None:
        assert a_out.dtype == torch.bfloat16 and a_out.stride(1) == 1 and tuple(a_out.shape) == (M, K) and Zin.dtype == torch.bfloat16
        a.a_out, a.lda_out = _p(a_out), a_out.stride(0)
    if drop is not None and drop[2] > 0.0:
        assert Zin.dtype == torch.bfloat16
        set_drop(a.drop, drop)
        a.drop_ld = N if drop_ld is None else drop_ld
        a.drop_col_div = int(drop_col_div)
    a.W, a.ldw, a.bias = _p(W), W.stride(0), _p(_f32(bias, "bias"))
    if R is not None:
        assert R.dtype == torch.bfloat16 and R.stride(1) == 1 and tuple(R.shape) == (M, N)
        a.R, a.ldr = _p(R), R.stride(0)
    a.out, a.ldo, a.out_dtype = _p(out), out.stride(0), dt_of(out)
    a.act, a.res_from_x, a.eps = act, 1 if res_from_x else 0, eps
    a.M, a.N, a.K = M, N, K
    _timed("dec_stage_kernel", 2.0 * M * N * K, float(M * K * Zin.element_size() * ((N + 31) // 32) + N * K * 2 + M * N * out.element_size()),
           lambda: check(lib().made_dec_stage(C.byref(a), _stream()), "made_dec_stage"), f"M={M} N={N} K={K}")
    return out


def attention(Q: Tensor, K: Tensor, V: Tensor, O: Tensor, H: int, *, key_mask: Optional[Tensor] = None,
              q_mask: Optional[Tensor] = None, scale: Optional[float] = None, Lk: Optional[int] = None,
              q_skip_mask: Optional[Tensor] = None, lse: Optional[Tensor] = None, drop=None,
              order: Optional[Tensor] = None, keep_bits: Optional[Tensor] = None) -> Tensor:
    assert Q.dim() == 3 and K.dim() == 3 and V.dim() == 3 and O.dim() == 3
    assert Q.stride(2) == 1 and K.stride(2) == 1 and V.stride(2) == 1 and O.stride(2) == 1
    assert Q.dtype == K.dtype == V.dtype == O.dtype
    B, Lq, D = Q.shape
    hd = D // H
    a = MadeAttnArgs()
    a.Q, a.K, a.V, a.O = _p(Q), _p(K), _p(V), _p(O)
    a.dtype, a.hd = dt_of(Q), hd
    a.B, a.H, a.Lq, a.Lk = B, H, Lq, (K.shape[1] if Lk is None else Lk)
    a.q_bs, a.ldq = Q.stride(0), Q.stride(1)
    a.k_bs, a.ldk = K.stride(0), K.stride(1)
    a.v_bs, a.ldv = V.stride(0), V.stride(1)
    a.o_bs, a.ldo = O.stride(0), O.stride(1)
    a.key_mask = _p(_f32(key_mask, "key_mask"))
    a.q_mask = _p(_f32(q_mask, "q_mask"))
    a.q_skip_mask = _p(_f32(q_skip_mask, "q_skip_mask"))
    a.scale = (1.0 / math.sqrt(hd)) if scale is None else scale
    if order is not None:
        assert order.dtype == torch.int32 and order.numel() == B and order.is_contiguous()
        a.batch_order = _p(order)
    if lse is not None:
        assert lse.dtype == torch.float32 and lse.is_contiguous() and lse.numel() == B * H * Lq
        a.lse = _p(lse)
    if drop is not None and drop[2] > 0.0:
        set_drop(a.drop, drop)
        if keep_bits is not None:
            assert keep_bits.dtype == torch.int32 and keep_bits.dim() == 2 and keep_bits.is_contiguous()
            assert keep_bits.shape[0] >= B * H * ((a.Lk + 31) // 32) and keep_bits.shape[1] >= Lq
            a.keep_bits, a.ld_bits = _p(keep_bits), keep_bits.shape[1]
    esz = 4 if a.dtype == F32 else 2
    flops = 4.0 * B * H * Lq * a.Lk * hd
    nbytes = esz * B * D * (2 * Lq + 2 * a.Lk)
    _timed("attention_" + ("f32" if a.dtype == F32 else "bf16"), flops, nbytes,
           lambda: check(lib().made_attention(C.byref(a), _stream()), "made_attention"),
           ("attn", key_mask, q_skip_mask) if (key_mask is not None and key_mask.dim() == 2) else f"B={B} H={H} hd={hd} Lq={Lq} Lk={a.Lk}")
    return O


def attention_bits_shape(B: int, H: int, Lq: int, Lk: int):
    return (B * H * ((Lk + 31) // 32), 32 * ((Lq + 31) // 32))


def attention_bits_decode(bits: Tensor, B: int, H: int, Lq: int, Lk: int) -> Tensor:
    nkt, ldq = (Lk + 31) // 32, bits.shape[1]
    w = bits[:B * H * nkt].view(B, H, nkt, ldq)
    q = torch.arange(Lq, device=bits.device)
    ql = q & 31
    slot = (q & ~31) + 2 * ((ql & 3) + 4 * (ql >> 3)) + ((ql >> 2) & 1)
    w = w[:, :, :, slot]
    b = (w[..., None] >> torch.arange(32, device=bits.device, dtype=torch.int32)) & 1
    return b.permute(0, 1, 3, 2, 4).reshape(B, H, Lq, nkt * 32)[..., :Lk].bool()


class WidePlan(NamedTuple):
    words: Tensor
    B: int
    L: int
    n_slots: int
    max_slices: int

    def header(self):
        return tuple(int(x) for x in self.words[:_lib.WIDE_PLAN_HEAD].tolist())

    def samples(self) -> Tensor:
        return self.words[_lib.WIDE_PLAN_HEAD:_lib.WIDE_PLAN_HEAD + _lib.WIDE_PLAN_SAMPLE * self.B].view(self.B, _lib.WIDE_PLAN_SAMPLE)

    def slots(self) -> Tensor:
        return self.words[_lib.WIDE_PLAN_HEAD + _lib.WIDE_PLAN_SAMPLE * self.B:][:_lib.WIDE_PLAN_SLOT * self.n_slots].view(self.n_slots, _lib.WIDE_PLAN_SLOT)


def wide_slice_plan(key_mask: Tensor, *, n_slots: int, max_slices: int = 8, order: Optional[Tensor] = None, out: Optional[Tensor] = None) -> WidePlan:
    assert key_mask.dim() == 2
    B, L = key_mask.shape
    words = _lib.wide_plan_words(B, n_slots)
    if out is None:
        out = torch.empty(words, device=key_mask.device, dtype=torch.int32)
    assert out.dtype == torch.int32 and out.is_contiguous() and out.numel() >= words
# ... 737 lines not shown
```

mgsv_amd/ops_train.py:

```python
from __future__ import annotations

import ctypes as C
from typing import Optional, Tuple

import torch

from . import _lib, tape as _tape
from ._lib import BF16, F32, MadeAttnBwdArgs, MadeDropout, MadeGemmTNArgs, MadeGemmTNGroup, check, lib
from .ops import _f32, _p, _stream, _timed, dt_of, set_drop

Tensor = torch.Tensor
Pair = Tuple[int, int]


_TN_WS_LIMIT = 1 << 32
_TN_SLAB_US = 1.3


def _tn_splits(tiles: int, nslab: int, gathered: bool, cap: int) -> int:
    if _lib.variant_env("MADE_TN_SPLIT_MODEL", "1") == "0":
        sp = max(8, (512 // max(tiles, 1)) // 8 * 8) if cap == 64 and tiles < 64 else max(1, 2048 // max(tiles, 1))
        while (nslab + sp - 1) // sp > 64:
            sp += 8
        return min(sp, max(1, nslab))
    live = max(1, (nslab * 9) // 16 if gathered else nslab)
    best, best_t = 1, float("inf")
    for sp in (1, 2, 3, 4, 6, 8, 16, 24, 32, 40, 48, 56, 64):
        if sp > max(1, cap) or sp > nslab:
            break
        if (nslab + sp - 1) // sp > 64:
            continue
        t = ((tiles * sp + 511) // 512) * ((live + sp - 1) // sp) * _TN_SLAB_US + tiles * sp * 0.0546
        if t < best_t:
            best, best_t = sp, t
    while (nslab + best - 1) // best > 64:
        best += 1 if best < 8 else 8
    return best


def gemm_tn(A: Tensor, B: Tensor, Cout: Tensor, *, alpha: float = 1.0, accumulate: bool = False, split_m: Optional[int] = None,
            row_mask: Optional[Tensor] = None, row_groups: Optional[Tensor] = None, rows=None, colsum: Optional[Tensor] = None,
            batch: Pair = (1, 1),
            a_zs: Pair = (0, 0), b_zs: Pair = (0, 0), c_zs: Pair = (0, 0), mask_zs: Pair = (0, 0),
            colsum_zs: Pair = (0, 0)) -> Tensor:
    M, N = A.shape
    K = B.shape[1]
    assert B.shape[0] == M and tuple(Cout.shape) == (N, K), (A.shape, B.shape, Cout.shape)
    assert A.stride(1) == 1 and B.stride(1) == 1 and Cout.stride(1) == 1
    assert A.dtype == B.dtype
    nz = batch[0] * batch[1]
    if split_m is None:
        split_m = 1
        if accumulate:
            slab = 64 if A.dtype == torch.bfloat16 else 32
            tiles = ((N + 127) // 128) * ((K + 127) // 128) * nz
            fast = A.dtype == torch.bfloat16 and N % 128 == 0 and K % 128 == 0 and nz == 1 and (row_mask is None or rows is not None)
            if fast:
                split_m = _tn_splits(tiles, (M + slab - 1) // slab, rows is not None, 64)
            else:
                split_m = max(1, min(512 // max(tiles, 1), ((M + slab - 1) // slab) // 8, 256))
    a = MadeGemmTNArgs()
    a.A, a.B, a.C = _p(A), _p(B), _p(Cout)
    a.ab_dtype, a.c_dtype = dt_of(A), dt_of(Cout)
    a.M, a.N, a.K = M, N, K
    a.lda, a.ldb, a.ldc = A.stride(0), B.stride(0), Cout.stride(0)
    a.batch1, a.batch2 = batch
    a.a_zs1, a.a_zs2 = a_zs
    a.b_zs1, a.b_zs2 = b_zs
    a.c_zs1, a.c_zs2 = c_zs
    a.row_mask = _p(_f32(row_mask, "row_mask"))
    a.row_group_valid = _p(_f32(row_groups, "row_groups")) if (row_mask is not None and nz == 1) else None
    if rows is not None and nz == 1:
        a.row_index, a.n_rows = _p(rows[0]), _p(rows[1])
    a.mask_zs1, a.mask_zs2 = mask_zs
    a.alpha, a.accumulate, a.split_m = float(alpha), int(bool(accumulate)), int(split_m)
    a.colsum = _p(_f32(colsum, "colsum"))
    a.colsum_zs1, a.colsum_zs2 = colsum_zs
    flops = 2.0 * M * N * K * nz
    nbytes = float((M * N + M * K) * A.element_size() * nz + N * K * Cout.element_size())
    _timed("made_gemm_tn", flops, nbytes, lambda: check(lib().made_gemm_tn(C.byref(a), _stream()), "made_gemm_tn"),
           ("rows", rows[1], M) if (rows is not None and nz == 1) else f"M={M} N={N} K={K} z={nz}")
    return Cout


def gemm_tn_grouped_workspace(device, nbytes: int) -> Tensor:
    return torch.empty(int(nbytes), dtype=torch.uint8, device=device)


def gemm_tn_grouped(problems, rows=None, alpha: float = 1.0, split_m: Optional[int] = None, workspace=None) -> None:
    assert 1 <= len(problems) <= 8
    M = problems[0][0].shape[0]
    g = MadeGemmTNGroup()
# ... 35 lines not shown
def row_groups(mask: Tensor, out: Optional[Tensor] = None) -> Tensor:
    m = mask.reshape(-1)
    M = m.numel()
    if out is None:
        out = torch.empty((M + 31) // 32, device=m.device, dtype=torch.float32)
    check(lib().made_row_groups(_p(_f32(m, "mask")), M, _p(out), _stream()), "made_row_groups")
    return out


def dropout_desc(seed: int, site: int, p: float) -> MadeDropout:
    d = MadeDropout()
    set_drop(d, (seed, site, p))
    return d


def attention_bwd(Q: Tensor, K: Tensor, V: Tensor, O: Tensor, dO: Tensor, dQ: Tensor, dK: Tensor, dV: Tensor, lse: Tensor,
                  delta: Tensor, H: int, *, key_mask: Optional[Tensor] = None, q_skip_mask: Optional[Tensor] = None,
                  scale: Optional[float] = None, drop=None, order: Optional[Tensor] = None, keep_bits: Optional[Tensor] = None) -> None:
    import math
    for t in (Q, K, V, O, dO, dQ, dK, dV):
        assert t.dim() == 3 and t.stride(2) == 1 and t.dtype == Q.dtype
    B, Lq, D = Q.shape
    hd = D // H
    a = MadeAttnBwdArgs()
    a.Q, a.K, a.V, a.O, a.dO, a.dQ, a.dK, a.dV = _p(Q), _p(K), _p(V), _p(O), _p(dO), _p(dQ), _p(dK), _p(dV)
    a.lse, a.delta = _p(_f32(lse, "lse")), _p(_f32(delta, "delta"))
    assert delta.numel() >= B * H * Lq
    a.dtype, a.hd = dt_of(Q), hd
    a.B, a.H, a.Lq, a.Lk = B, H, Lq, K.shape[1]
    a.q_bs, a.ldq, a.k_bs, a.ldk, a.v_bs, a.ldv = Q.stride(0), Q.stride(1), K.stride(0), K.stride(1), V.stride(0), V.stride(1)
    a.o_bs, a.ldo, a.do_bs, a.lddo = O.stride(0), O.stride(1), dO.stride(0), dO.stride(1)
    a.dq_bs, a.lddq, a.dk_bs, a.lddk, a.dv_bs, a.lddv = dQ.stride(0), dQ.stride(1), dK.stride(0), dK.stride(1), dV.stride(0), dV.stride(1)
    a.key_mask = _p(_f32(key_mask, "key_mask"))
    a.q_skip_mask = _p(_f32(q_skip_mask, "q_skip_mask"))
    if order is not None:
        assert order.dtype == torch.int32 and order.numel() == a.B and order.is_contiguous()
        a.batch_order = _p(order)
    a.scale = (1.0 / math.sqrt(hd)) if scale is None else scale
    if drop is not None and drop[2] > 0.0:
        set_drop(a.drop, drop)
        if keep_bits is not None:
            assert keep_bits.dtype == torch.int32 and keep_bits.dim() == 2 and keep_bits.is_contiguous()
            assert keep_bits.shape[0] >= B * H * ((a.Lk + 31) // 32) and keep_bits.shape[1] >= Lq
            a.keep_bits, a.ld_bits = _p(keep_bits), keep_bits.shape[1]
    flops = 10.0 * B * H * Lq * a.Lk * hd
    _timed("made_attention_bwd", flops, float(Q.element_size() * B * D * (4 * Lq + 4 * a.Lk)),
           lambda: check(lib().made_attention_bwd(C.byref(a), _stream()), "made_attention_bwd"),
           ("attn", key_mask, q_skip_mask) if (key_mask is not None and key_mask.dim() == 2) else f"B={B} H={H} hd={hd} Lq={Lq} Lk={a.Lk}")


def _drop_ptr(drop):
    if drop is None or drop[2] <= 0.0:
        return None
    return C.byref(dropout_desc(*drop))


def _dt(t: Optional[Tensor]) -> int:
    return dt_of(t) if t is not None else F32


def layernorm_bwd(x: Tensor, gamma: Tensor, dy: Tensor, dx: Tensor, *, dgamma: Optional[Tensor], dbeta: Optional[Tensor],
                  add: Optional[Tensor] = None, dx_drop: Optional[Tensor] = None, drop=None, drop_ld: int = 0,
                  row_skip: Optional[Tensor] = None, eps: float = 1e-5) -> Tensor:
    if x.dim() == 3:
        rpb, xbs, ldx = x.shape[1], x.stride(0), x.stride(1)
        rows, D = x.shape[0] * x.shape[1], x.shape[2]
    else:
        rpb, xbs, ldx = 0, 0, x.stride(0)
        rows, D = x.shape
    assert dy.dim() == 2 and dx.dim() == 2 and dy.shape[0] == rows and dx.shape[0] == rows
    check(lib().made_layernorm_bwd(_p(x), dt_of(x), ldx, rpb, xbs, _p(_f32(gamma, "gamma")), _p(dy), dt_of(dy), dy.stride(0),
                                   _p(add), _dt(add), add.stride(0) if add is not None else 0,
                                   _p(dx), dt_of(dx), dx.stride(0),
                                   _p(dx_drop), dx_drop.stride(0) if dx_drop is not None else 0, _drop_ptr(drop), drop_ld,
                                   _p(_f32(dgamma, "dgamma")), _p(_f32(dbeta, "dbeta")), rows, D, eps,
                                   _p(_f32(row_skip, "row_skip")), _stream()), "made_layernorm_bwd")
    return dx


def dec_stage_bwd(xa: Tensor, gamma_a: Tensor, dy: Tensor, W: Tensor, out: Tensor, *, dgamma_a: Optional[Tensor], dbeta_a: Optional[Tensor],
                  xb: Optional[Tensor] = None, gamma_b: Optional[Tensor] = None, dgamma_b: Optional[Tensor] = None, dbeta_b: Optional[Tensor] = None,
                  add: Optional[Tensor] = None, dx_out: Optional[Tensor] = None, a_out: Optional[Tensor] = None, drop_a=None,
                  G: Optional[Tensor] = None, gate_scale: float = 1.0, drop_o=None, drop_o_ld: int = 0, drop_o_col_div: int = 1,
                  R: Optional[Tensor] = None, eps: float = 1e-5) -> Tensor:
    from . import _lib as L
    M, K = xa.shape
    N = W.shape[0]
    for t in (xa, dy, xb, add, dx_out, a_out, W, G, R, out):
        assert t is None or (t.dim() == 2 and t.dtype == torch.bfloat16 and t.stride(1) == 1)
    assert W.shape[1] == K and tuple(out.shape) == (M, N)
    a = L.MadeDecStageBwdArgs()
    a.xa, a.gamma_a, a.ldxa = _p(xa), _p(_f32(gamma_a, "gamma_a")), xa.stride(0)
    if xb is not None:
        a.xb, a.gamma_b, a.ldxb = _p(xb), _p(_f32(gamma_b, "gamma_b")), xb.stride(0)
    a.dy, a.lddy = _p(dy), dy.stride(0)
    if add is not None:
        a.add, a.ldadd = _p(add), add.stride(0)
    if dx_out is not None:
        a.dx_out, a.lddx = _p(dx_out), dx_out.stride(0)
    if a_out is not None:
        a.a_out, a.lda_out = _p(a_out), a_out.stride(0)
    a.dgamma_a, a.dbeta_a = _p(_f32(dgamma_a, "dgamma_a")), _p(_f32(dbeta_a, "dbeta_a"))
    a.dgamma_b, a.dbeta_b = _p(_f32(dgamma_b, "dgamma_b")), _p(_f32(dbeta_b, "dbeta_b"))
    if drop_a is not None and drop_a[2] > 0.0:
        set_drop(a.drop_a, drop_a)
    a.drop_a_ld = K
    a.W, a.ldw = _p(W), W.stride(0)
    if G is not None:
        a.G, a.ldg = _p(G), G.stride(0)
    a.gate_scale, a.eps = float(gate_scale), float(eps)
    if drop_o is not None and drop_o[2] > 0.0:
        set_drop(a.drop_o, drop_o)
    a.drop_o_ld, a.drop_o_col_div = (drop_o_ld or N), int(drop_o_col_div)
    if R is not None:
        a.R, a.ldr = _p(R), R.stride(0)
    a.out, a.ldo = _p(out), out.stride(0)
    a.M, a.N, a.K = M, N, K
    _timed("dec_stage_bwd_kernel", 2.0 * M * N * K, float(M * K * 2 * 2 * ((N + 31) // 32) + N * K * 2 + M * N * 2),
           lambda: check(lib().made_dec_stage_bwd(C.byref(a), _stream()), "made_dec_stage_bwd"), f"M={M} N={N} K={K}")
    return out


def layernorm_bwd2(xa: Tensor, gamma_a: Tensor, xb: Tensor, gamma_b: Tensor, dy: Tensor, dx: Tensor, *, dgamma_a: Tensor, dbeta_a: Tensor,
                   dgamma_b: Tensor, dbeta_b: Tensor, add: Optional[Tensor] = None, dx_drop: Optional[Tensor] = None, drop=None,
                   drop_ld: int = 0, eps: float = 1e-5) -> Tensor:
    rows, D = xa.shape
    for t in (xa, xb, dy, dx, add, dx_drop):
        assert t is None or (t.dim() == 2 and t.dtype == xa.dtype and t.stride(1) == 1 and t.shape[0] >= rows)
    check(lib().made_layernorm_bwd2(_p(xa), _p(_f32(gamma_a, "gamma_a")), xa.stride(0), _p(xb), _p(_f32(gamma_b, "gamma_b")), xb.stride(0),
                                    _p(dy), dy.stride(0), _p(add), add.stride(0) if add is not None else 0, _p(dx), dx.stride(0),
                                    _p(dx_drop), dx_drop.stride(0) if dx_drop is not None else 0, _drop_ptr(drop), drop_ld, dt_of(xa),
                                    _p(_f32(dgamma_a, "dgamma_a")), _p(_f32(dbeta_a, "dbeta_a")), _p(_f32(dgamma_b, "dgamma_b")),
                                    _p(_f32(dbeta_b, "dbeta_b")), rows, D, eps, _stream()), "made_layernorm_bwd2")
    return dx


def pool_bwd(mean: Tensor, dvec: Tensor, mask: Tensor, out: Tensor, in1: Optional[Tensor] = None, in2: Optional[Tensor] = None,
             eps: float = 1e-12) -> Tensor:
    B, T, D = out.shape
    def bs(t): return (t.stride(0), t.stride(1)) if t is not None else (0, 0)
    check(lib().made_pool_bwd(_p(_f32(mean, "mean")), _p(_f32(dvec, "dvec")), _p(_f32(mask, "mask")),
                              _p(in1), _dt(in1), *bs(in1), _p(in2), _dt(in2), *bs(in2),
                              _p(out), dt_of(out), *bs(out), B, T, D, eps, _stream()), "made_pool_bwd")
    return out


def l2norm_bwd(x: Tensor, dy: Tensor, dx: Optional[Tensor] = None, *, accumulate: bool = False, dx_alt: Optional[Tensor] = None,
               eps: float = 1e-12, dy_rows_per: int = 1) -> None:
    rows, D = x.shape
    check(lib().made_l2norm_bwd(_p(x), dt_of(x), x.stride(0), _p(_f32(dy, "dy")), dy.stride(0), dy_rows_per,
                                _p(dx), dx.stride(0) if dx is not None else 0, int(accumulate),
                                _p(dx_alt), _dt(dx_alt), dx_alt.stride(0) if dx_alt is not None else 0,
                                rows, D, eps, _stream()), "made_l2norm_bwd")


def clip_loss_bwd(sims: Tensor, logit_scale: Tensor, weight: float, upstream: Optional[Tensor], lse_ws: Tensor, dsims: Tensor,
                  dsims_t: Optional[Tensor], d_logit_scale: Optional[Tensor], accumulate: bool = False,
                  row_exclude: Optional[Tensor] = None) -> None:
    n = sims.shape[0]
    assert lse_ws.numel() >= 2 * n and dsims.is_contiguous()
    assert row_exclude is None or (row_exclude.shape == sims.shape and row_exclude.is_contiguous())
    check(lib().made_clip_loss_bwd(_p(_f32(sims, "sims")), sims.stride(0), n, _p(logit_scale), float(weight), _p(upstream),
                                   _p(lse_ws), _p(dsims), _p(dsims_t), int(accumulate), _p(d_logit_scale),
                                   _p(_f32(row_exclude, "row_exclude")), _stream()),
          "made_clip_loss_bwd")


def xpool_tail_bwd(y: Tensor, gamma: Tensor, beta: Tensor, video: Tensor, dsims: Tensor, dy: Tensor, Nm: int, Nv: int, *,
                   dy_drop: Optional[Tensor] = None, drop=None, dgamma: Optional[Tensor] = None, dbeta: Optional[Tensor] = None,
                   dvideo: Optional[Tensor] = None, dpool: Optional[Tensor] = None, dpool_scale: float = 1.0, eps: float = 1e-5) -> None:
    D = y.shape[1]
    check(lib().made_xpool_tail_bwd(_p(y), dt_of(y), y.stride(0), _p(gamma), _p(beta), _p(_f32(video, "video")), video.stride(0),
                                    _p(_f32(dsims, "dsims")), dsims.stride(0), _p(dy), dt_of(dy), dy.stride(0), _p(dy_drop),
                                    _drop_ptr(drop), _p(dgamma), _p(dbeta), _p(dvideo), dvideo.stride(0) if dvideo is not None else 0,
                                    _p(_f32(dpool, "dpool")), dpool.stride(0) if dpool is not None else 0, float(dpool_scale),
                                    Nm, Nv, D, eps, _stream()), "made_xpool_tail_bwd")


def softmax_bwd(S: Tensor, dP: Tensor, mask: Optional[Tensor], rows_per_mask: int, scale: float, Pd: Tensor, dS: Tensor,
                dSt: Optional[Tensor], rows_per_batch: int, L: int, *, extra: Optional[Tensor] = None, drop=None,
                ldo: Optional[int] = None, ldt: int = 0, out_batch_stride: int = 0, t_batch_stride: int = 0) -> None:
    rows = S.shape[0]
    check(lib().made_softmax_bwd(_p(_f32(S, "S")), S.stride(0), _p(dP), dP.stride(0), _p(mask), rows_per_mask,
                                 _p(extra), float(scale), _drop_ptr(drop), _p(Pd), _p(dS), _p(dSt), dt_of(Pd),
                                 Pd.stride(-2) if ldo is None else ldo, ldt, out_batch_stride, t_batch_stride,
                                 rows, rows_per_batch, L, _stream()), "made_softmax_bwd")


def attention_wide_bwd(Q: Tensor, dO: Tensor, O: Tensor, K: Tensor, V: Tensor, lse: Tensor, Pd: Tensor, dS: Tensor, dQ: Tensor, *, scale: float,
                       key_mask: Optional[Tensor] = None, ssum: Optional[Tensor] = None, extra: Optional[Tensor] = None,
                       dattc: Optional[Tensor] = None, vbias: Optional[Tensor] = None, hd: int = 0, drop=None, n_split: int = 1,
                       part_dq: Optional[Tensor] = None, plan=None) -> Tensor:
    assert Q.dim() == 3 and dO.shape == Q.shape and O.shape == Q.shape and dQ.shape == Q.shape and K.dim() == 3 and V.shape == K.shape
    B, NQ, D = Q.shape
    L = K.shape[1]
    for t in (Q, dO, O, K, V, Pd, dS, dQ):
        assert t.dtype == torch.bfloat16 and t.stride(-1) == 1
    assert Pd.dim() == 3 and dS.dim() == 3 and Pd.stride() == dS.stride() and Pd.shape[0] == B and Pd.shape[1] == NQ
    a = _lib.MadeWideAttnBwdArgs()
    a.Q, a.dO, a.O, a.K, a.V = _p(Q), _p(dO), _p(O), _p(K), _p(V)
# ... 92 lines not shown
```

mgsv_amd/trainer.py:

```python
from __future__ import annotations

import contextlib
import ctypes as C
import functools
import math
import os
import struct
from typing import Dict, List, Optional, Tuple

import numpy as np
import torch

from . import _lib, dropout as dr, ops, ops_train as tr, tape as _tape
from .config import MadeConfig
from .engine import MadeEngine
from .ops import Seg, round_up

WIDE_SLICES = 8

Tensor = torch.Tensor
XA = "video_guided_to_music_pooling_cross_transformer"


HEAD_PAD = 64
# ... 655 lines not shown
            ops.attention(q3[:, :, :D], q3[:, :, D:2 * D], q3[:, :, 2 * D:], att.view(B, L, D), H, key_mask=fus_mask,
                          q_skip_mask=qskip, lse=tw[e + ".lse"], drop=self._drop(f"enc.{l}" + ".attn", pd),
                          order=self._order[fus_mask.data_ptr()], keep_bits=tw[e + ".kbits"] if self._bits else None)
            x = ops.linear(att, P[p + ".out.w"], P[p + ".out.b"], R=xin if pre else src, out=tw[e + ".x"], rows=rows_f,
                           drop=self._drop(f"enc.{l}" + ".drop1", pd))
            s1 = ops.layernorm(x, P[p + (".ln2.g" if pre else ".ln1.g")], P[p + (".ln2.b" if pre else ".ln1.b")], out=tw[e + ".s1"], row_skip=fskip)
            h = ops.linear(s1, P[p + ".ff1.w"], P[p + ".ff1.b"], act=ops.ACT_RELU, out=tw[e + ".h"], rows=rows_f,
                           drop=self._drop(f"enc.{l}" + ".ffn_act", pd))
            x2 = ops.linear(h, P[p + ".ff2.w"], P[p + ".ff2.b"], R=x if pre else s1, out=tw[e + ".x2"], rows=rows_f,
                            drop=self._drop(f"enc.{l}" + ".drop2", pd))
            last = l == c.detr_enc_layers - 1
            if pre:
                xin = x2
                if last:
                    ops.layernorm_add(x2, P["enc.norm.g"], P["enc.norm.b"], pos2, tw["mem"], tw["mempos"], row_skip=fskip)
                continue
            nsrc, nsp = (tw["mem"], tw["mempos"]) if last else (tw[f"e.{l + 1}.src"], tw[f"e.{l + 1}.srcpos"])
            ops.layernorm_add(x2, P[p + ".ln2.g"], P[p + ".ln2.b"], pos2, nsrc, nsp, row_skip=fskip)
        return tw["mem"].view(B, L, D)

    def _query_pos_rows(self) -> Tensor:
        B, Q, qp = self._shape[0], self.cfg.num_moment_queries, self.P["query_embed"]
        return qp.expand(B * Q, self.cfg.D) if Q == 1 else qp.repeat(B, 1)

    def _dec_fill_tgt(self, ws, tw) -> None:
        c = self.cfg
        B, Q, D = self._shape[0], c.num_moment_queries, c.D
        tgt = tw["d.0.tgt"]
        if c.moment_query_type in ("video", "music", "xpool"):
            src_vec = {"video": ws["video"], "music": ws["music"], "xpool": tw["xpool_q"]}[c.moment_query_type]
            if Q == 1:
                tr.add3(tgt, src_vec)
            else:
                tgt.view(B, Q, D).copy_(src_vec[:, None, :].expand(B, Q, D))
        else:
            _tape.zero_(tgt)
        if Q > 1 and not c.detr_pre_norm:
            tr.add3(tw["d.0.tq"], tgt, self.P["query_embed"], b_mod=Q * D)

    def _dec_self_attn_fwd(self, tw, l: int, x: Tensor) -> None:
        c, P = self.cfg, self.P
        B, D, Q, H = self._shape[0], c.D, c.num_moment_queries, c.detr_nheads
        p, d = f"detr_transformer.decoder.layers.{l}", f"d.{l}"
        Wsa, bsa = P[p + ".sa.in.w"], P[p + ".sa.in.b"]
        drop = self._drop(f"dec.{l}" + ".sa_attn", float(c.detr_dropout))
        if Q == 1:
            ops.linear(x, Wsa[2 * D:], bsa[2 * D:], out=tw[d + ".att"], drop=drop, drop_ld=H, drop_col_div=D // H)
            return
        qkv = tw[d + ".qkv"]
        ops.linear(x, Wsa, bsa, A2=tw[d + ".tq"], a2_replace=True,
                   segs=[Seg(out=qkv, col_begin=0, use_a2=True), Seg(out=qkv[:, 2 * D:], col_begin=2 * D, ldo=qkv.stride(0))])
        q3 = qkv.view(B, Q, 3 * D)
        ops.attention(q3[:, :, :D], q3[:, :, D:2 * D], q3[:, :, 2 * D:], tw[d + ".att"].view(B, Q, D), H, lse=tw[d + ".lse"], drop=drop)

    def _dec_query_side(self, tw, l: int) -> None:
        c, P = self.cfg, self.P
        B, D, Q, H = self._shape[0], c.D, c.num_moment_queries, c.detr_nheads
        hd, pd = D // H, float(c.detr_dropout)
        p, d = f"detr_transformer.decoder.layers.{l}", f"d.{l}"
        tgt, qp = tw[d + ".tgt"], P["query_embed"]
        Win, bin_ = P[p + ".ca.in.w"], P[p + ".ca.in.b"]
        Wt = P[p + ".ca.in.wt"]
        stage, pre = self._dec_stage_chain(), bool(c.detr_pre_norm)
        if stage:
            Wsa, bsa = P[p + ".sa.in.w"], P[p + ".sa.in.b"]
            sa_drop = dict(drop=self._drop(f"dec.{l}" + ".sa_attn", pd), drop_ld=H, drop_col_div=hd)
            if l == 0:
                ops.dec_stage(tgt, Wsa[2 * D:], bsa[2 * D:], tw[d + ".att"], **sa_drop)
            else:
                q_ = f"detr_transformer.decoder.layers.{l - 1}"
                ops.dec_stage(tw[f"d.{l - 1}.t_c"], Wsa[2 * D:], bsa[2 * D:], tw[d + ".att"], ln=(P[q_ + ".ln3.g"], P[q_ + ".ln3.b"]),
                              x_out=tgt, **sa_drop)
        elif pre:
            n1 = tw[d + ".n1"]
            qp_rows = self._query_pos_rows()
            if Q == 1:
                ops.layernorm(tgt, P[p + ".ln1.g"], P[p + ".ln1.b"], out=n1)
            else:
                ops.layernorm_add(tgt, P[p + ".ln1.g"], P[p + ".ln1.b"], qp_rows, n1, tw[d + ".tq"])
            self._dec_self_attn_fwd(tw, l, n1)
        else:
            self._dec_self_attn_fwd(tw, l, tgt)
        ta = ops.linear(tw[d + ".att"], P[p + ".sa.out.w"], P[p + ".sa.out.b"], R=tgt, out=tw[d + ".t_a"], drop=self._drop(f"dec.{l}" + ".drop1", pd))
        if stage:
            qc = ops.dec_stage(ta, Win[:D], bin_[:D], tw[d + ".qc"], ln=(P[p + ".ln1.g"], P[p + ".ln1.b"]), add=qp,
                               x_out=tw[d + ".t1"], a_out=tw[d + ".t1q"])
        else:
            ln = ".ln2" if pre else ".ln1"
            ops.layernorm_add(ta, P[p + ln + ".g"], P[p + ln + ".b"], qp_rows if pre else self._query_pos_rows(), tw[d + ".t1"], tw[d + ".t1q"])
            qc = ops.linear(tw[d + ".t1q"], Win[:D], bin_[:D], out=tw[d + ".qc"])
        qprime = tw["GQ"][:, 1, l]
        ops.linear(qc[:, :hd], Wt[:, D:D + hd], None, M=B * Q, N=D, K=hd, batch=H, a_z_stride=hd, w_z_stride=hd,
                   segs=[Seg(out=qprime, ldo=D, rows_per_batch=Q, out_batch_stride=qprime.stride(0), out_z_stride=Q * D)])

    def _decoder_fwd(self, ws, tw) -> Dict[str, Tensor]:
        c, P = self.cfg, self.P
        B, L = self._shape[0], self._fused_len()
        D, Q, nd, H = c.D, c.num_moment_queries, c.detr_dec_layers, c.detr_nheads
        hd, pd = D // H, float(c.detr_dropout)
        ca_scale = 1.0 / math.sqrt(hd)
        fus_mask, hs = ws["fus_mask"], ws["hs"]
        mem3, mempos3 = tw["mem"].view(B, L, D), tw["mempos"].view(B, L, D)
        stage = self._dec_stage_chain()
        n_split, wplan = self._wide_split(B)
        for l in range(nd):
            p, d = f"detr_transformer.decoder.layers.{l}", f"d.{l}"
            if l > 0:
                self._dec_query_side(tw, l)
            Win, bin_ = P[p + ".ca.in.w"], P[p + ".ca.in.b"]
            qprime, t1 = tw["GQ"][:, 1, l], tw[d + ".t1"]
            pooled = tw[d + ".pooled"]
            s_out = tw[d + ".s"] if Q == 1 else tw["s_raw"]
            ops.attention_wide(qprime.view(B, H, Q, D), mempos3, mem3, pooled.view(B, Q, H, D).permute(0, 2, 1, 3), scale=ca_scale,
                               key_mask=fus_mask, drop=self._drop(f"dec.{l}" + ".ca_attn", pd), sum_out=s_out,
                               n_split=n_split, part_o=ws["part_o"], part_ml=ws["part_ml"],
                               lse_out=tw["ca_lse"][l] if stage else None, plan=wplan)
            if Q > 1:
                tw[d + ".s"].view(B, Q, H).copy_(s_out.view(B, H, Q).permute(0, 2, 1))
            attc = tw[d + ".attc"]
            if stage:
                ops.linear(pooled[:, :D], Win[2 * D:2 * D + hd], bin_[2 * D:], M=B * Q, N=hd, K=D, batch=H, a_z_stride=D, w_z_stride=hd * D,
                           segs=[Seg(out=attc, ldo=D, out_z_stride=hd)], bias_row_scale=tw[d + ".s"], bias_z_stride=hd)
            else:
                ops.linear(pooled[:, :D], Win[2 * D:2 * D + hd], None, M=B * Q, N=hd, K=D, batch=H, a_z_stride=D, w_z_stride=hd * D,
                           segs=[Seg(out=attc, ldo=D, out_z_stride=hd)])
                tr.head_bias(attc, tw[d + ".s"], bin_[2 * D:], H)
            if c.detr_pre_norm:
                tb = ops.linear(attc, P[p + ".ca.out.w"], P[p + ".ca.out.b"], R=tw[d + ".t_a"], out=tw[d + ".t_b"], drop=self._drop(f"dec.{l}" + ".drop2", pd))
                t2 = ops.layernorm(tb, P[p + ".ln3.g"], P[p + ".ln3.b"], out=tw[d + ".t2"])
                h = ops.linear(t2, P[p + ".ff1.w"], P[p + ".ff1.b"], act=ops.ACT_RELU, out=tw[d + ".h"], drop=self._drop(f"dec.{l}" + ".ffn_act", pd))
                ops.linear(h, P[p + ".ff2.w"], P[p + ".ff2.b"], R=tb, out=tw[d + ".t3"], drop=self._drop(f"dec.{l}" + ".drop3", pd))
                continue
            tb = ops.linear(attc, P[p + ".ca.out.w"], P[p + ".ca.out.b"], R=t1, out=tw[d + ".t_b"], drop=self._drop(f"dec.{l}" + ".drop2", pd))
            if stage:
                h = ops.dec_stage(tb, P[p + ".ff1.w"], P[p + ".ff1.b"], tw[d + ".h"], ln=(P[p + ".ln2.g"], P[p + ".ln2.b"]), x_out=tw[d + ".t2"],
                                  act=ops.ACT_RELU, drop=self._drop(f"dec.{l}" + ".ffn_act", pd))
                t2 = tw[d + ".t2"]
            else:
                t2 = ops.layernorm(tb, P[p + ".ln2.g"], P[p + ".ln2.b"], out=tw[d + ".t2"])
                h = ops.linear(t2, P[p + ".ff1.w"], P[p + ".ff1.b"], act=ops.ACT_RELU, out=tw[d + ".h"], drop=self._drop(f"dec.{l}" + ".ffn_act", pd))
            tcx = ops.linear(h, P[p + ".ff2.w"], P[p + ".ff2.b"], R=t2, out=tw[d + ".t_c"], drop=self._drop(f"dec.{l}" + ".drop3", pd))
            t3 = tw[d + ".t3"]
            if stage:
                if l + 1 == nd:
                    ops.layernorm(tcx, P[p + ".ln3.g"], P[p + ".ln3.b"], out=t3)
            elif l + 1 < nd:
                ops.layernorm_add(tcx, P[p + ".ln3.g"], P[p + ".ln3.b"], self._query_pos_rows(), t3, tw[f"d.{l + 1}.tq"])
            else:
                ops.layernorm(tcx, P[p + ".ln3.g"], P[p + ".ln3.b"], out=t3)
        ops.layernorm(tw["dstack"]["tgt"][1:].reshape(nd * B * Q, D), P["dec.norm.g"], P["dec.norm.b"], out=hs.view(nd * B * Q, D))
        return dict(hs=hs.view(nd, B, Q, D))

    def _heads_fwd(self, ws, tw, v_duration: Optional[Tensor]) -> Dict[str, Tensor]:
        c, P = self.cfg, self.P
        B, Tv, _ = self._shape
        D, Q, nd = c.D, c.num_moment_queries, c.detr_dec_layers
        hs, music, frame = ws["hs"], ws["music"], self._views[0]
        out: Dict[str, Tensor] = {}
        hs2 = hs.view(nd * B * Q, D)
        logits, spans = ws["logits"], ws["spans"]
        ops.linear(hs2, P["class_embed.w"], P["class_embed.b"], out=logits.view(-1, 2))
        h1 = ops.linear(hs2, P["span_embed.0.w"], P["span_embed.0.b"], act=ops.ACT_RELU, out=tw["h1"])
        h2 = ops.linear(h1, P["span_embed.1.w"], P["span_embed.1.b"], act=ops.ACT_RELU, out=tw["h2"])
        if c.predict_center == 1:
            ops.linear(h2, P["span_embed.2.w"], P["span_embed.2.b"], act=ops.ACT_SIGMOID, segs=[Seg(out=spans.view(-1, 2), ldo=2)])
            spans[..., 1] = (v_duration.to(self.device, torch.float32) / c.max_m_duration).view(1, B, 1)
        else:
            ops.linear(h2, P["span_embed.2.w"], P["span_embed.2.b"], act=ops.ACT_SIGMOID, out=spans.view(-1, 2))
        out.update(pred_logits=logits[-1], pred_spans=spans[-1], logits_all=logits, spans_all=spans)
        if c.moment_loss:
            last = hs[nd - 1]
            m1 = ops.linear(last, P["moment_embed.0.w"], P["moment_embed.0.b"], act=ops.ACT_RELU)
            m2 = ops.linear(m1, P["moment_embed.1.w"], P["moment_embed.1.b"], act=ops.ACT_RELU)
            m3 = ops.linear(m2, P["moment_embed.2.w"], P["moment_embed.2.b"], out_dtype=torch.float32)
            mf = ops.l2norm_rows(m3)
            if c.audio_short_cut:
                mq = music if Q == 1 else music[:, None, :].expand(B, Q, D).contiguous()
                tr.add3(m3, mf, mq, b_mod=B * Q * D)
                mf = ops.l2norm_rows(m3)
            out["moment_feats"] = mf.view(B, Q, D)
        pq = vid_sum = None
        if c.contrastive_align_loss:
            ops.linear(hs2, P["proj_q.w"], P["proj_q.b"], out=ws["pq_raw"])
            pq = ws["pq"]
            pq2 = pq.view(nd * B * Q, -1)
            if c.audio_short_cut:
                mq = music if Q == 1 else music[:, None, :].expand(B, Q, D).contiguous()
                ops.l2norm_rows(ws["pq_raw"], out_f32=tw["pq_n0"])
                tr.add3(tw["pq_s1"], tw["pq_n0"], mq, b_mod=B * Q * D)
                ops.l2norm_rows(tw["pq_s1"], out_f32=pq2)
                if c.aux_loss and nd > 1:
                    n_aux = (nd - 1) * B * Q
                    tr.add3(tw["pq_s2"][:n_aux], pq2[:n_aux], mq, b_mod=B * Q * D)
                    ops.l2norm_rows(tw["pq_s2"][:n_aux], out_f32=pq2[:n_aux])
            else:
                ops.l2norm_rows(ws["pq_raw"], out_f32=pq2)
            self._frame_rows_linear(frame, P["proj_v.w"], P["proj_v.b"], ws["pv_raw"], B, Tv)
            pv = ws["pv"]
            ops.l2norm_rows(ws["pv_raw"], out_f32=pv.view(B * Tv, pq.shape[-1]))
            vid_sum = ops.masked_mean(pv, None, out=ws["vid_sum"])
            out.update(proj_queries=pq[-1], proj_vid_mem=pv, proj_queries_all=pq)
        tg = self._inputs[4]
        pi, ti, cnt, status, cost = ops.hungarian_match(logits.view(nd * B, Q, 2), spans.view(nd * B, Q, 2), tg, c.foreground_label)
        losses, total = ops.set_criterion(logits, spans, tg, pi, ti, cnt, pq, vid_sum, P["empty_weight"], c.foreground_label, P["crit_weights"])
        self._match = (pi, ti, cnt)
        out.update(matcher_pred_idx=pi.view(nd, B, -1), matcher_tgt_idx=ti.view(nd, B, -1), matcher_count=cnt.view(nd, B),
                   matcher_status=status, criterion_losses=losses, localization_loss=total)
        return out

    def _opt_stream(self):
        st = getattr(self, "_opt_st", None)
        if st is None:
            st = self._opt_st = torch.cuda.Stream(device=self.device)
        return st

    def _wide_slots(self) -> int:
        if getattr(self, "_wide_slots_n", None) is None:
            self._wide_slots_n = max(8, min(1024, _lib.device_info()[1]))
        return self._wide_slots_n

    def _wide_planned_ok(self, B: int, HQ: int, D: int) -> bool:
        return self.tc == torch.bfloat16 and D in (256, 512) and HQ <= 32 and B <= self._wide_slots()

    def _wide_split(self, B: int, backward: bool = False):
        plan = self._wide_plan
        if backward and self.cfg.detr_nheads * self.cfg.num_moment_queries > 8:
            plan = None
        if plan is not None:
            return WIDE_SLICES, plan
        return max(1, min(8, 256 // max(B, 1))), None

    def _dec_stage_chain(self) -> bool:
        c = self.cfg
        return (self.tc == torch.bfloat16 and c.num_moment_queries == 1 and c.D in (256, 512) and not c.detr_pre_norm
                and _lib.variant_env("MADE_DEC_STAGE", "1") != "0")

    def _encode_train(self, feats: Tensor, mask: Tensor, which: str, ws, tw, row_off: int) -> None:
        c, P = self.cfg, self.P
        if c.agg_module == "mlp":
            return self._encode_train_mlp(feats, mask, which, ws, tw, row_off)
        B, T, Kin = feats.shape
        D, Hh = c.D, c.SA_temporal_heads
        proj, mod, pe, depth, tag = (("vit_proj", "video_transformer", "pe_video", c.video_transformer_depth, "v") if which == "video"
                                     else ("ast_proj", "audio_transformer", "pe_audio", c.audio_transformer_depth, "a"))
        cls = bool(c.with_cls_token)
        T1 = T + 1 if cls else T
        if P[pe].shape[0] < T1:
            raise ValueError(f"{which} position table holds {P[pe].shape[0]} positions < {T1}")
        nrow = B * T
        mflat = mask.reshape(-1)
        pt = dr.P_TEMPORAL
        name = "video" if which == "video" else "audio"
        act = ops.ACT_QUICKGELU if c.with_act_after_proj else ops.ACT_NONE
        zp = tw[tag + ".zproj"] if c.with_act_after_proj else None
        x = tw[f"{tag}.0.x0"]
        if cls:
            mask1 = tw[tag + ".mask1"]
            mask1[:, 0] = 1.0; mask1[:, 1:] = mask
            self._index_lists(mask1, tw[tag + ".rows1"], tw[tag + ".order1"])
            x3 = x.view(B, T1, D)
            x3[:, 0] = (P["cls_" + name].float() + P[pe][0].float()).to(self.tc)
            lin_out = dict(segs=[Seg(out=x3[:, 1:], ldo=D, rows_per_batch=T, out_batch_stride=T1 * D)])
            pe_rows = P[pe][1:T1]
        else:
            mask1 = mask
            lin_out = dict(out=x, rows=self._rw(mflat))
            pe_rows = P[pe][:T]
        mflat1 = mask1.reshape(-1)
        rws = self._rw(mflat1)
        if self.tc == torch.bfloat16:
            xin = ops.cast_mask_rows(feats.view(nrow, Kin), mflat, tw[tag + ".xin"])
            ops.linear(xin, P[proj + ".w"], P[proj + ".b"], act=act, Zout=zp, R=pe_rows, r_row_mod=T, **lin_out)
        else:
            ops.linear(feats.view(nrow, Kin), P[proj + ".w"], P[proj + ".b"], a_row_mask=mflat, act=act, Zout=zp, R=pe_rows, r_row_mod=T, **lin_out)
        for l in range(depth):
            p, t = f"{mod}.layers.{l}", f"{tag}.{l}"
            x1 = ops.layernorm(x, P[p + ".ln1.g"], P[p + ".ln1.b"], out=tw[t + ".x1"], row_skip=mflat1)
            qkv = ops.linear(x1, P[p + ".in.w"], P[p + ".in.b"], out=tw[t + ".qkv"], rows=rws)
            q3 = qkv.view(B, T1, 3 * D)
            att = tw[t + ".att"]
            ops.attention(q3[:, :, :D], q3[:, :, D:2 * D], q3[:, :, 2 * D:], att.view(B, T1, D), Hh, key_mask=mask1, q_skip_mask=mask1,
                          lse=tw[t + ".lse"], drop=self._drop(f"{name}.{l}.attn", pt), order=self._order[mask1.data_ptr()],
                          keep_bits=tw[t + ".kbits"] if self._bits else None)
            x2 = ops.linear(att, P[p + ".out.w"], P[p + ".out.b"], R=x1, out=tw[t + ".x2"], rows=rws)
            x3_ = ops.layernorm(x2, P[p + ".ln2.g"], P[p + ".ln2.b"], out=tw[t + ".x3"], row_skip=mflat1)
            h = ops.linear(x3_, P[p + ".ff1.w"], P[p + ".ff1.b"], act=ops.ACT_GELU, out=tw[t + ".h"], Zout=tw[t + ".z1"], rows=rws,
                           drop=self._drop(f"{name}.{l}.ffn_act", pt))
            nxt = tw[f"{tag}.{l + 1}.x0"] if l + 1 < depth else tw[tag + ".xlast"]
            x = ops.linear(h, P[p + ".ff2.w"], P[p + ".ff2.b"], R=x3_, out=nxt, rows=rws, drop=self._drop(f"{name}.{l}.ffn_out", pt))
        if "concat" in c.mml_fusion:
            local = ws["fus"][:, row_off:row_off + T]
        else:
            local = ws["frame_buf"] if which == "video" else ws["seg_buf"]
        vec = ws["video"] if which == "video" else ws["music"]
        if cls:
            y3 = ops.linear(x, P[mod + ".final.w"], P[mod + ".final.b"], out_row_mask=mflat1, out=tw[tag + ".y1"]).view(B, T1, D)
            ops.l2norm_rows(y3[:, 0], out_f32=vec)
            local.copy_(y3[:, 1:])
            return
        ops.linear(x, P[mod + ".final.w"], P[mod + ".final.b"], out_row_mask=mflat, tile_skip_mask=mflat,
                   segs=[Seg(out=local, ldo=local.stride(1), rows_per_batch=T, out_batch_stride=local.stride(0))])
        ops.masked_mean(local, mask, out=tw[tag + ".mean"])
        ops.l2norm_rows(tw[tag + ".mean"], out_f32=vec)

    def _xpool_train(self, video: Tensor, seg: Tensor, seg_mask: Optional[Tensor], ws, tw, B: int, S: int, key: str = "xa", pre: str = "x",
                     sims_out: Optional[Tensor] = None) -> None:
        P, D = self.P, self.cfg.D
        skip = seg_mask.reshape(-1) if seg_mask is not None else None
        v1 = ops.layernorm(video, P[key + ".ln1.g"], P[key + ".ln1.b"], out=tw[pre + "v1"])
        q = ops.linear(v1, P[key + ".q.w"], P[key + ".q.b"], out=tw[pre + "q"])
        s1 = ops.layernorm(seg, P[key + ".ln1.g"], P[key + ".ln1.b"], out=tw[pre + "s1"], row_skip=skip)
        ops.linear(s1, P[key + ".kv.w"], P[key + ".kv.b"], rows=self._rw(skip), tile_skip_mask=skip if self._rw(skip) is None else None,
                   segs=[Seg(out=tw[pre + "k"], col_begin=0), Seg(out=tw[pre + "u"], col_begin=D)])
        inbatch = (self.tc == torch.bfloat16 and B <= 64 and S <= 512 and S * D >= 65536 and D in (256, 512) and _lib.variant_env("MADE_XPOOL_INBATCH", "1") != "0")
        if inbatch:
            if tw.get(pre + "xib_ws") is None or tw[pre + "xib_ws"].numel() < ops.xpool_inbatch_ws_bytes(B, S):
                tw[pre + "xib_ws"] = torch.zeros(ops.xpool_inbatch_ws_bytes(B, S), device=self.device, dtype=torch.uint8)
            ops.xpool_inbatch(q, tw[pre + "k"].view(B, S, D), tw[pre + "u"].view(B, S, D), seg_mask, tw[pre + "o"].view(B, B, D),
                              scale=1.0 / math.sqrt(D), ws=tw[pre + "xib_ws"])
# ... 221 lines not shown
            self._lin_bwd(tw["dpq_raw"], hs2, "proj_q", dx_out=dhs, R=dhs, later=heads_dw)
            tr.l2norm_bwd(ws["pv_raw"], tw["dvid_sum"], dx_alt=tw["dpv_raw"], dy_rows_per=Tv)
            heads_dw.append(lambda: tr.gemm_tn(tw["dpv_raw"][:Tv], frame[0], G["proj_v.w"], accumulate=True, colsum=G["proj_v.b"], batch=(B, 1),
                                               a_zs=(Tv * Dc, 0), b_zs=(frame.stride(0), 0), colsum_zs=(0, 0)))
            ops.linear(tw["dpv_raw"], P["proj_v.wt"], None, out=tw["dframe_x"])
        return heads_dw

    def _fused_len(self) -> int:
        _, Tv, Ta = self._shape
        return Tv + Ta if "concat" in self.cfg.mml_fusion else Ta

    def _dec_self_attn_bwd(self, tw, l: int, g_sa: Tensor, gqkv: Tensor, g4: Tensor, dx_out: Tensor, R: Optional[Tensor] = None) -> Tensor:
        c, P, G = self.cfg, self.P, self.G
        B, D, Q, H = self._shape[0], c.D, c.num_moment_queries, c.detr_nheads
        p, d = f"detr_transformer.decoder.layers.{l}", f"d.{l}"
        datt = ops.linear(g_sa, P[p + ".sa.out.wt"], None, out=g4)
        q3, g3v = tw[d + ".qkv"].view(B, Q, 3 * D), gqkv.view(B, Q, 3 * D)
        tr.attention_bwd(q3[:, :, :D], q3[:, :, D:2 * D], q3[:, :, 2 * D:], tw[d + ".att"].view(B, Q, D), datt.view(B, Q, D),
                         g3v[:, :, :D], g3v[:, :, D:2 * D], g3v[:, :, 2 * D:], tw[d + ".lse"], tw["d_delta"], H,
                         drop=self._drop(f"dec.{l}" + ".sa_attn", float(c.detr_dropout)))
        dx = ops.linear(gqkv, P[p + ".sa.in.wt"], None, R=R, out=dx_out)
        dqk = ops.linear(gqkv[:, :2 * D], P[p + ".sa.in.wt"][:, :2 * D], None, out=g4)
        tr.colsum(dqk.view(B, Q * D), G["query_embed"].view(-1))
        return dx

    def _decoder_bwd(self, ws, tw) -> Tuple[Tensor, Tensor]:
        c, P, G = self.cfg, self.P, self.G
        B, L = self._shape[0], self._fused_len()
        D, Q, nd, H = c.D, c.num_moment_queries, c.detr_dec_layers, c.detr_nheads
        hd, HQ = D // H, H * Q
        pd = float(c.detr_dropout)
        inv_keep = 1.0 / (1.0 - pd) if (self.training_dropout and pd > 0) else 1.0
        fus_mask, dhs = ws["fus_mask"], tw["dhs"]
        mem3, mempos3 = tw["mem"].view(B, L, D), tw["mempos"].view(B, L, D)
        Lp = tw["PdS"].shape[-1]
        GQ, PdS = tw["GQ"], tw["PdS"]
        ca_scale = 1.0 / math.sqrt(hd)
        st = tw["dstack"]
        dtgt = None
        stage = self._dec_stage_chain()
        pre = bool(c.detr_pre_norm)
        if stage:
            n_split, wplan = self._wide_split(B, backward=True)
            gN = tw["dgN"]
            tr.layernorm_bwd(st["tgt"][1:].reshape(nd * B * Q, D), P["dec.norm.g"], dhs, gN, dgamma=G["dec.norm.g"], dbeta=G["dec.norm.b"])
        else:
            S_all = tw["dS_S"]
            ops.linear(GQ[0, 1].reshape(nd * HQ, D), mempos3[0], None, M=nd * HQ, N=L, K=D, batch=B, a_z_stride=GQ.stride(0), w_z_stride=L * D,
                       segs=[Seg(out=S_all, ldo=Lp, rows_per_batch=HQ, out_batch_stride=B * HQ * Lp, out_z_stride=HQ * Lp)])
        for l in range(nd - 1, -1, -1):
            p, d = f"detr_transformer.decoder.layers.{l}", f"d.{l}"
            g1, g2, g4 = tw["dg1"], tw["dg2"], tw["dg4"]
            if stage:
                ch = tw["dchain"][l]
                g1a, g1b, g2a, g2b, g2c, dt_out = ch[0], ch[1], ch[2], ch[3], ch[4], ch[5]
            else:
                g1a = g1b = g1
                g2a = g2b = g2
            Win, Wt = P[p + ".ca.in.w"], P[p + ".ca.in.wt"]
            g_ffn, g_z, g_ca, g_attc, g_q, g_qc, g_sa, gqkv = (st[k][l] for k in ("g_ffn", "g_z", "g_ca", "g_attc", "g_q", "g_qc", "g_sa", "g_qkv"))
            if stage:
                tr.dec_stage_bwd(tw[d + ".t_c"], P[p + ".ln3.g"], gN[l * B * Q:(l + 1) * B * Q], P[p + ".ff2.wt"], g_z,
                                 dgamma_a=G[p + ".ln3.g"], dbeta_a=G[p + ".ln3.b"], add=dtgt, dx_out=g2a, a_out=g_ffn,
                                 drop_a=self._drop(f"dec.{l}" + ".drop3", pd), G=tw[d + ".h"], gate_scale=inv_keep)
            elif pre:
                tr.layernorm_bwd(tw[d + ".t3"], P["dec.norm.g"], dhs[l * B * Q:(l + 1) * B * Q], g1, dgamma=G["dec.norm.g"], dbeta=G["dec.norm.b"], add=dtgt)
                tr.gate_rows(g1, g_ffn, drop=self._drop(f"dec.{l}" + ".drop3", pd))
            else:
                tr.layernorm_bwd(tw[d + ".t3"], P["dec.norm.g"], dhs[l * B * Q:(l + 1) * B * Q], g1, dgamma=G["dec.norm.g"], dbeta=G["dec.norm.b"], add=dtgt)
                tr.layernorm_bwd(tw[d + ".t_c"], P[p + ".ln3.g"], g1, g2, dgamma=G[p + ".ln3.g"], dbeta=G[p + ".ln3.b"],
                                 dx_drop=g_ffn, drop=self._drop(f"dec.{l}" + ".drop3", pd))
            if not stage:
                ops.linear(g_ffn, P[p + ".ff2.wt"], None, out=g_z, gate=_lib.GATE_RELU_OUT, G=tw[d + ".h"], gate_scale=inv_keep)
            if pre:
                dn3 = ops.linear(g_z, P[p + ".ff1.wt"], None, out=g4)
                tr.layernorm_bwd(tw[d + ".t_b"], P[p + ".ln3.g"], dn3, g2, dgamma=G[p + ".ln3.g"], dbeta=G[p + ".ln3.b"], add=g1,
                                 dx_drop=g_ca, drop=self._drop(f"dec.{l}" + ".drop2", pd))
                dattc = ops.linear(g_ca, P[p + ".ca.out.wt"], None, out=g_attc)
            else:
                dt2 = ops.linear(g_z, P[p + ".ff1.wt"], None, out=g1a, R=g2a)
            if pre:
                pass
            elif stage:
                dattc = tr.dec_stage_bwd(tw[d + ".t_b"], P[p + ".ln2.g"], dt2, P[p + ".ca.out.wt"], g_attc, dgamma_a=G[p + ".ln2.g"],
                                         dbeta_a=G[p + ".ln2.b"], dx_out=g2b, a_out=g_ca, drop_a=self._drop(f"dec.{l}" + ".drop2", pd))
            else:
                tr.layernorm_bwd(tw[d + ".t_b"], P[p + ".ln2.g"], dt2, g2, dgamma=G[p + ".ln2.g"], dbeta=G[p + ".ln2.b"],
                                 dx_drop=g_ca, drop=self._drop(f"dec.{l}" + ".drop2", pd))
                dattc = ops.linear(g_ca, P[p + ".ca.out.wt"], None, out=g_attc)
            dpooled = GQ[:, 0, l]
            qprime = GQ[:, 1, l]
            if stage:
                ops.linear(dattc[:, :hd], Wt[:, 2 * D:2 * D + hd], None, M=B * Q, N=D, K=hd, batch=H, a_z_stride=hd, w_z_stride=hd,
                           segs=[Seg(out=dpooled, ldo=D, rows_per_batch=Q, out_batch_stride=dpooled.stride(0), out_z_stride=Q * D)])
                tr.attention_wide_bwd(qprime, dpooled, tw[d + ".pooled"].view(B, HQ, D), mempos3, mem3, tw["ca_lse"][l].view(B, HQ),
                                      PdS[:, 0, l], PdS[:, 1, l], g_q, scale=ca_scale, key_mask=fus_mask, ssum=tw[d + ".s"].view(B, HQ),
                                      dattc=dattc, vbias=P[p + ".ca.in.b"][2 * D:], hd=hd, drop=self._drop(f"dec.{l}" + ".ca_attn", pd),
                                      n_split=n_split, part_dq=ws["part_o"], plan=wplan)
            else:
                tr.head_bias_bwd(dattc, tw[d + ".s"], P[p + ".ca.in.b"][2 * D:], G[p + ".ca.in.b"][2 * D:], tw["d_ds"], H)
                d_ds = tw["d_ds"]
                if Q > 1:
                    tw["dds_raw"].view(B, H, Q).copy_(d_ds.view(B, Q, H).permute(0, 2, 1))
                    d_ds = tw["dds_raw"]
                ops.linear(dattc[:, :hd], Wt[:, 2 * D:2 * D + hd], None, M=B * Q, N=D, K=hd, batch=H, a_z_stride=hd, w_z_stride=hd,
                           segs=[Seg(out=dpooled, ldo=D, rows_per_batch=Q, out_batch_stride=dpooled.stride(0), out_z_stride=Q * D)])
                S, dP = S_all[l], tw["dS_dP"]
                ops.linear(dpooled[0], mem3[0], None, M=HQ, N=L, K=D, batch=B, a_z_stride=dpooled.stride(0), w_z_stride=L * D,
                           segs=[Seg(out=dP, ldo=Lp, out_z_stride=HQ * Lp)])
                tr.softmax_bwd(S, dP, fus_mask, HQ, ca_scale, PdS[:, 0, l], PdS[:, 1, l], tw["dSt"], HQ, L, extra=d_ds.view(-1),
                               drop=self._drop(f"dec.{l}" + ".ca_attn", pd), ldo=Lp, ldt=HQ, out_batch_stride=PdS.stride(0))
                gq_out = g_q if Q == 1 else tw["gq_raw"]
                tr.gemm_tn(tw["dSt"][0], mempos3[0], gq_out[0], batch=(B, 1), a_zs=(L * HQ, 0), b_zs=(L * D, 0), c_zs=(HQ * D, 0),
                           row_mask=fus_mask, mask_zs=(L, 0))
                if Q > 1:
                    g_q.view(B, Q, H, D).copy_(gq_out.view(B, H, Q, D).permute(0, 2, 1, 3))
            dq2 = g_q.view(B * Q, H * D)
            ops.linear(dq2[:, :D], Win[D:D + hd], None, M=B * Q, N=hd, K=D, batch=H, a_z_stride=D, w_z_stride=hd * D,
                       segs=[Seg(out=g_qc, ldo=D, out_z_stride=hd)])
            dt1q = st["dt1q"][l]
            if pre:
                ops.linear(g_qc, Wt[:, :D], None, out=dt1q)
                tr.layernorm_bwd(tw[d + ".t_a"], P[p + ".ln2.g"], dt1q, g1, dgamma=G[p + ".ln2.g"], dbeta=G[p + ".ln2.b"], add=g2,
                                 dx_drop=g_sa, drop=self._drop(f"dec.{l}" + ".drop1", pd))
                if Q == 1:
                    ops.linear(g_sa, P[p + ".sa.out.wt"], None, segs=[Seg(out=gqkv[:, 2 * D:], ldo=gqkv.stride(0))],
                               drop=self._drop(f"dec.{l}" + ".sa_attn", pd), drop_ld=H, drop_col_div=hd)
                    dn1 = ops.linear(gqkv[:, 2 * D:], P[p + ".sa.in.wt"][:, 2 * D:], None, out=g4)
                else:
                    dn1 = self._dec_self_attn_bwd(tw, l, g_sa, gqkv, g4, dx_out=g2)
                dtgt = tr.layernorm_bwd(tw[d + ".tgt"], P[p + ".ln1.g"], dn1, tw["dtgt"], dgamma=G[p + ".ln1.g"], dbeta=G[p + ".ln1.b"], add=g1)
                continue
            ops.linear(g_qc, Wt[:, :D], None, out=g1b, R=g2b, Zout=dt1q)
            if stage:
                tr.dec_stage_bwd(tw[d + ".t_a"], P[p + ".ln1.g"], g1b, P[p + ".sa.out.wt"], gqkv[:, 2 * D:], dgamma_a=G[p + ".ln1.g"],
                                 dbeta_a=G[p + ".ln1.b"], dx_out=g2c, a_out=g_sa, drop_a=self._drop(f"dec.{l}" + ".drop1", pd),
                                 drop_o=self._drop(f"dec.{l}" + ".sa_attn", pd), drop_o_ld=H, drop_o_col_div=hd)
                dtgt = ops.linear(gqkv[:, 2 * D:], P[p + ".sa.in.wt"][:, 2 * D:], None, R=g2c, out=dt_out)
                continue
            tr.layernorm_bwd(tw[d + ".t_a"], P[p + ".ln1.g"], g1, g2, dgamma=G[p + ".ln1.g"], dbeta=G[p + ".ln1.b"],
                             dx_drop=g_sa, drop=self._drop(f"dec.{l}" + ".drop1", pd))
            if Q == 1:
                ops.linear(g_sa, P[p + ".sa.out.wt"], None, segs=[Seg(out=gqkv[:, 2 * D:], ldo=gqkv.stride(0))],
                           drop=self._drop(f"dec.{l}" + ".sa_attn", pd), drop_ld=H, drop_col_div=hd)
                dtgt = ops.linear(gqkv[:, 2 * D:], P[p + ".sa.in.wt"][:, 2 * D:], None, R=g2, out=tw["dtgt"])
            else:
                dtgt = self._dec_self_attn_bwd(tw, l, g_sa, gqkv, g4, dx_out=tw["dtgt"], R=g2)
        dmem = tw["eg1"]
        tr.gemm_tn(PdS.view(B, 2 * nd * HQ, Lp)[0, :, :L], GQ.view(B, 2 * nd * HQ, D)[0], dmem.view(B, L, D)[0], batch=(B, 1),
                   a_zs=(PdS.stride(0), 0), b_zs=(GQ.stride(0), 0), c_zs=(L * D, 0))
        return dmem, dtgt

    def _decoder_dw(self, tw, heads_dw: list) -> None:
        c, P, G = self.cfg, self.P, self.G
        B, D, Q, nd, H = self._shape[0], c.D, c.num_moment_queries, c.detr_dec_layers, c.detr_nheads
        hd, BQ = D // H, B * Q
        st = tw["dstack"]
        for launch in heads_dw:
            launch()
        tr.colsum(st["dt1q"].view(nd * B, Q * D), G["query_embed"].view(-1))
        if self._dec_stage_chain():
            for l in range(nd):
                pl = f"detr_transformer.decoder.layers.{l}"
                tr.head_bias_bwd(st["g_attc"][l], tw[f"d.{l}.s"], P[pl + ".ca.in.b"][2 * D:], G[pl + ".ca.in.b"][2 * D:], tw["d_ds"], H)
        p0, p1 = "detr_transformer.decoder.layers.0", "detr_transformer.decoder.layers.1"

        def lstride(key):
            return (G[p1 + key].data_ptr() - G[p0 + key].data_ptr()) // 4 if nd > 1 else 0

        def batched(a_stack, b_stack, wkey, bkey, a_cols=None, b_cols=None, w_rows=None):
            A, Bm = a_stack[0], b_stack[0]
            if a_cols is not None:
                A = A[:, a_cols[0]:a_cols[1]]
            if b_cols is not None:
                Bm = Bm[:, b_cols[0]:b_cols[1]]
            gw, gb = G[p0 + wkey], (G[p0 + bkey] if bkey is not None else None)
            if w_rows is not None:
# ... 551 lines not shown
```

Before: 14230 pairs/s.

## Fold per-head projection GEMM into decoder stage kernels

Adds fold variants of the decoder stage forward and backward kernels. Each block computes a full head's slice of the stage GEMM output, keeps it in shared memory, and multiplies it by the per-head weight slice with 32x32 MFMA to write the projected query (forward) or pooled gradient (backward) directly. This removes a separate batched linear launch and its intermediate round trip through memory. In exchange, the stage GEMM is recomputed once per N2 slice, and the fold is enabled by default only in the forward pass for the last few decoder layers.

```diff
diff --git a/include/made_hip.h b/include/made_hip.h
--- a/include/made_hip.h
+++ b/include/made_hip.h
@@ -160,6 +160,13 @@
     int64_t M, N, K;
 } MadeDecStageBwdArgs;
 int made_dec_stage_bwd(const MadeDecStageBwdArgs* args, void* stream);
+
+typedef struct MadeDecFold {
+    const void* W2; int64_t ldw2; int64_t w2_z_stride; int64_t N2;
+    void* out2; int64_t ldo2; int64_t out2_z_stride; int64_t hd;
+} MadeDecFold;
+int made_dec_stage_fold(const MadeDecStageArgs* args, const MadeDecFold* fold, void* stream);
+int made_dec_stage_bwd_fold(const MadeDecStageBwdArgs* args, const MadeDecFold* fold, void* stream);
 
 typedef struct MadeFinishArgs {
     const float* ws; int64_t split_k, M, N;
diff --git a/mgsv_amd/_lib.py b/mgsv_amd/_lib.py
--- a/mgsv_amd/_lib.py
+++ b/mgsv_amd/_lib.py
@@ -86,6 +86,10 @@
                 ("W", vp), ("ldw", i64), ("G", vp), ("ldg", i64), ("gate_scale", f32), ("eps", f32),
                 ("drop_o", MadeDropout), ("drop_o_ld", i64), ("drop_o_col_div", i32), ("_pad", i32),
                 ("R", vp), ("ldr", i64), ("out", vp), ("ldo", i64), ("M", i64), ("N", i64), ("K", i64)]
+
+
+class MadeDecFold(C.Structure):
+    _fields_ = [("W2", vp), ("ldw2", i64), ("w2_z_stride", i64), ("N2", i64), ("out2", vp), ("ldo2", i64), ("out2_z_stride", i64), ("hd", i64)]
 
 
 class MadeAttnArgs(C.Structure):
@@ -243,6 +247,8 @@
     "made_splitk_finish": (C.c_int, [C.POINTER(MadeFinishArgs), vp]),
     "made_dec_stage": (C.c_int, [C.POINTER(MadeDecStageArgs), vp]),
     "made_dec_stage_bwd": (C.c_int, [C.POINTER(MadeDecStageBwdArgs), vp]),
+    "made_dec_stage_fold": (C.c_int, [C.POINTER(MadeDecStageArgs), C.POINTER(MadeDecFold), vp]),
+    "made_dec_stage_bwd_fold": (C.c_int, [C.POINTER(MadeDecStageBwdArgs), C.POINTER(MadeDecFold), vp]),
     "made_attention": (C.c_int, [C.POINTER(MadeAttnArgs), vp]),
     "made_attention_wide": (C.c_int, [C.POINTER(MadeWideAttnArgs), vp]),
     "made_attention_wide_bwd": (C.c_int, [C.POINTER(MadeWideAttnBwdArgs), vp]),
diff --git a/mgsv_amd/csrc/decoder.hip b/mgsv_amd/csrc/decoder.hip
--- a/mgsv_amd/csrc/decoder.hip
+++ b/mgsv_amd/csrc/decoder.hip
@@ -4,30 +4,92 @@
 namespace {
 
 constexpr int DS_BM = 16, DS_BN = 16, DS_THREADS = 256, DS_RPW = 4, DS_CT_LD = DS_BN + 4;
+constexpr int DS_SL = 128;
 
 __device__ __forceinline__ float ds_act(float x, int act) {
     return act == MADE_ACT_RELU ? fmaxf(x, 0.f) : x;
 }
 
-template <int NV, bool ZB16, bool TRAIN>
-__global__ __launch_bounds__(DS_THREADS) void dec_stage_kernel(const MadeDecStageArgs a) {
+template <int NC>
+__device__ __forceinline__ void ds_fold_load(const void* W2, int64_t ldw2, int64_t w2_z_stride, int h, int n2, int hh, bf16x8 (&fw2)[NC]) {
+    const bf16_t* pw2 = (const bf16_t*)W2 + (int64_t)h * w2_z_stride + (int64_t)n2 * ldw2 + hh * 8;
+#pragma unroll
+    for (int c = 0; c < NC; ++c) fw2[c] = *(const bf16x8*)(pw2 + c * 16);
+}
+template <int NC>
+__device__ __forceinline__ void ds_fold_product(const bf16_t* q2, const bf16x8 (&fw2)[NC], void* out2, int64_t ldo2, int64_t out2_z_stride,
+                                                int h, int n2, int r32, int hh, int m0, int M) {
+    constexpr int DS_Q2_LD = NC * 16 + 8;
+    f32x16 p[NC];
+#pragma unroll
+    for (int c = 0; c < NC; ++c) {
+        const bf16x8 fa = *(const bf16x8*)(q2 + (r32 & 15) * DS_Q2_LD + c * 16 + hh * 8);
+#pragma unroll
+        for (int e = 0; e < 16; ++e) p[c][e] = 0.f;
+        p[c] = __builtin_amdgcn_mfma_f32_32x32x16_bf16(fa, fw2[c], p[c], 0, 0, 0);
+    }
+    bf16_t* op = (bf16_t*)out2 + (int64_t)h * out2_z_stride + n2;
+#pragma unroll
+    for (int e = 0; e < 8; ++e) {
+        const int ml = m0 + acc_row(e, hh);
+        float v = 0.f;
+#pragma unroll
+        for (int c = 0; c < NC; ++c) v += p[c][e];
+        if (ml < M) op[(int64_t)ml * ldo2] = (bf16_t)v;
+    }
+}
+
+__device__ __forceinline__ void ds_dropout8(const MadeDecStageArgs& a, int ml, int n, float (&v8)[8]) {
+    if (a.drop.p > 0.f) {
+        const uint32_t thr = made_drop_threshold(a.drop.p);
+        const float sc = 1.f / (1.f - a.drop.p);
+        const uint64_t seed = made_drop_seed(a.drop);
+        const uint64_t rb = (uint64_t)ml * (uint64_t)a.drop_ld;
+        const int div = a.drop_col_div > 1 ? a.drop_col_div : 1;
+        if (div == 1) {
+            const uint32_t kb = made_keep_bits<8>(seed, a.drop.site, thr, rb + (uint64_t)n);
+#pragma unroll
+            for (int j = 0; j < 8; ++j) v8[j] = ((kb >> j) & 1u) ? v8[j] * sc : 0.f;
+        } else {
+#pragma unroll
+            for (int j = 0; j < 8; ++j)
+                v8[j] = (made_rng_mix(seed, a.drop.site, rb + (uint64_t)((n + j) / div)) >> 8) >= thr ? v8[j] * sc : 0.f;
+        }
+    }
+}
+
+template <int NV, bool ZB16, bool TRAIN, int HD = 0>
+__global__ __launch_bounds__(DS_THREADS) void dec_stage_kernel(const MadeDecStageArgs a, const MadeDecFold f) {
+    constexpr bool FOLD = HD > 0;
+    constexpr int DS_HD = FOLD ? HD : DS_BN, DS_FT = DS_HD / DS_BN, DS_FCT_LD = DS_HD + 4, DS_Q2_LD = DS_HD + 8, NC = FOLD ? HD / 16 : 1;
     constexpr int K = 64 * NV;
     constexpr int LDA = K * 2 + 16;
     constexpr int STEPS = NV / 2;
+    constexpr int FT = FOLD ? DS_FT : 1;
     __shared__ __attribute__((aligned(16))) unsigned char dlds[DS_BM * LDA];
-    __shared__ __attribute__((aligned(16))) float Ct[4 * DS_BM * DS_CT_LD];
+    __shared__ __attribute__((aligned(16))) float Ct[4 * DS_BM * (FOLD ? DS_FCT_LD : DS_CT_LD)];
+    __shared__ __attribute__((aligned(16))) bf16_t q2[FOLD ? DS_BM * DS_Q2_LD : 8];
     const int tid = threadIdx.x;
     const int lane = tid & 63, wave = __builtin_amdgcn_readfirstlane(tid >> 6);
     const int r16 = lane & 15, kq = lane >> 4;
     const int M = (int)a.M, N = (int)a.N;
-    const int n0 = blockIdx.x * DS_BN, m0 = blockIdx.y * DS_BM;
+    const int heads = FOLD ? N / DS_HD : 1;
+    const int fh = FOLD ? (int)blockIdx.x % heads : 0, fslice = FOLD ? (int)blockIdx.x / heads : 0;
+    const int n0 = FOLD ? fh * DS_HD : blockIdx.x * DS_BN, m0 = blockIdx.y * DS_BM;
+    const int r32 = lane & 31, hh = lane >> 5;
+    const int n2 = fslice * DS_SL + wave * 32 + r32;
+    bf16x8 fw2[NC];
+    if constexpr (FOLD) ds_fold_load<NC>(f.W2, f.ldw2, f.w2_z_stride, fh, n2, hh, fw2);
 
     const int kw = wave * (K / 4) + kq * 8;
-    int gn = n0 + r16; gn = gn < N ? gn : N - 1;
-    const bf16_t* pw = (const bf16_t*)a.W + (int64_t)gn * a.ldw + kw;
-    bf16x8 fw[STEPS];
-#pragma unroll
-    for (int s = 0; s < STEPS; ++s) fw[s] = *(const bf16x8*)(pw + s * 32);
+    bf16x8 fw[FT][STEPS];
+#pragma unroll
+    for (int t = 0; t < FT; ++t) {
+        int gn = n0 + t * DS_BN + r16; gn = gn < N ? gn : N - 1;
+        const bf16_t* pw = (const bf16_t*)a.W + (int64_t)gn * a.ldw + kw;
+#pragma unroll
+        for (int s = 0; s < STEPS; ++s) fw[t][s] = *(const bf16x8*)(pw + s * 32);
+    }
 
     constexpr int RPW = DS_RPW;
     const int c0 = NV * lane;
@@ -150,7 +212,7 @@
             *(bf16x4*)(dlds + rl * LDA + c0 * 2) = t;
         }
     }
-    const int cc = tid & 1, row = (tid >> 1) & 15;
+    const int cc = FOLD ? (tid & (DS_HD / 8 - 1)) : (tid & 1), row = FOLD ? ((tid / (DS_HD / 8)) & 15) : ((tid >> 1) & 15);
     const int n = n0 + cc * 8;
     int nvalid = N - n; nvalid = nvalid > 8 ? 8 : nvalid;
     const int ml = m0 + row;
@@ -189,12 +251,14 @@
     }
     __syncthreads();
 
-    f32x4 acc;
-    acc[0] = acc[1] = acc[2] = acc[3] = 0.f;
+    f32x4 acc[FT];
+#pragma unroll
+    for (int t = 0; t < FT; ++t) acc[t][0] = acc[t][1] = acc[t][2] = acc[t][3] = 0.f;
 #pragma unroll
     for (int s = 0; s < STEPS; ++s) {
         const bf16x8 fa = *(const bf16x8*)(dlds + r16 * LDA + (kw + s * 32) * 2);
-        acc = __builtin_amdgcn_mfma_f32_16x16x32_bf16(fa, fw[s], acc, 0, 0, 0);
+#pragma unroll
+        for (int t = 0; t < FT; ++t) acc[t] = __builtin_amdgcn_mfma_f32_16x16x32_bf16(fa, fw[t][s], acc[t], 0, 0, 0);
     }
 
     float xres[8];
@@ -205,10 +269,41 @@
 #pragma unroll
         for (int j = 0; j < 8; ++j) xres[j] = (float)t[j];
     }
+    if constexpr (FOLD) {
+        float* mine = Ct + wave * (DS_BM * DS_FCT_LD);
+#pragma unroll
+        for (int t = 0; t < FT; ++t)
+#pragma unroll
+            for (int e = 0; e < 4; ++e) mine[(kq * 4 + e) * DS_FCT_LD + t * DS_BN + r16] = acc[t][e];
+        __syncthreads();
+        if (tid < 2 * DS_HD) {
+            float v8[8];
+#pragma unroll
+            for (int j = 0; j < 8; ++j) v8[j] = 0.f;
+#pragma unroll
+            for (int w = 0; w < 4; ++w) {
+                const float* cp = Ct + w * (DS_BM * DS_FCT_LD) + row * DS_FCT_LD + cc * 8;
+                const f32x4 q0 = *(const f32x4*)cp, q1 = *(const f32x4*)(cp + 4);
+                v8[0] += q0[0]; v8[1] += q0[1]; v8[2] += q0[2]; v8[3] += q0[3];
+                v8[4] += q1[0]; v8[5] += q1[1]; v8[6] += q1[2]; v8[7] += q1[3];
+            }
+            bf16x8 o;
+#pragma unroll
+            for (int j = 0; j < 8; ++j) v8[j] = ds_act(v8[j] + bv[j], a.act);
+            ds_dropout8(a, mlc, n, v8);
+#pragma unroll
+            for (int j = 0; j < 8; ++j) { v8[j] += 0.f; o[j] = (bf16_t)v8[j]; }
+            *(bf16x8*)(q2 + row * DS_Q2_LD + cc * 8) = o;
+            if (fslice == 0 && ml < M) *(bf16x8*)((bf16_t*)a.out + (int64_t)ml * a.ldo + n) = o;
+        }
+        __syncthreads();
+        ds_fold_product<NC>(q2, fw2, f.out2, f.ldo2, f.out2_z_stride, fh, n2, r32, hh, m0, M);
+        return;
+    }
     {
         float* mine = Ct + wave * (DS_BM * DS_CT_LD);
 #pragma unroll
-        for (int e = 0; e < 4; ++e) mine[(kq * 4 + e) * DS_CT_LD + r16] = acc[e];
+        for (int e = 0; e < 4; ++e) mine[(kq * 4 + e) * DS_CT_LD + r16] = acc[0][e];
     }
     __syncthreads();
     if (tid >= 32 || nvalid <= 0 || ml >= M) return;
@@ -237,24 +332,7 @@
     const int act = a.act;
 #pragma unroll
     for (int j = 0; j < 8; ++j) v8[j] = ds_act(v8[j] + bv[j], act);
-    if constexpr (TRAIN) {
-        if (a.drop.p > 0.f) {
-            const uint32_t thr = made_drop_threshold(a.drop.p);
-            const float sc = 1.f / (1.f - a.drop.p);
-            const uint64_t seed = made_drop_seed(a.drop);
-            const uint64_t rb = (uint64_t)ml * (uint64_t)a.drop_ld;
-            const int div = a.drop_col_div > 1 ? a.drop_col_div : 1;
-            if (div == 1) {
-                const uint32_t kb = made_keep_bits<8>(seed, a.drop.site, thr, rb + (uint64_t)n);
-#pragma unroll
-                for (int j = 0; j < 8; ++j) v8[j] = ((kb >> j) & 1u) ? v8[j] * sc : 0.f;
-            } else {
-#pragma unroll
-                for (int j = 0; j < 8; ++j)
-                    v8[j] = (made_rng_mix(seed, a.drop.site, rb + (uint64_t)((n + j) / div)) >> 8) >= thr ? v8[j] * sc : 0.f;
-            }
-        }
-    }
+    if constexpr (TRAIN) ds_dropout8(a, ml, n, v8);
 #pragma unroll
     for (int j = 0; j < 8; ++j) v8[j] += rv[j];
     if (a.out_dtype == MADE_F32) {
@@ -320,30 +398,43 @@
     else { bf16x4 t; for (int u = 0; u < 4; ++u) t[u] = (bf16_t)v[u]; *(bf16x4*)((bf16_t*)p + off) = t; }
 }
 
-template <int NV, int MODE>
-__global__ __launch_bounds__(DS_THREADS) void dec_stage_bwd_kernel(const MadeDecStageBwdArgs a) {
+template <int NV, int MODE, int HD = 0>
+__global__ __launch_bounds__(DS_THREADS) void dec_stage_bwd_kernel(const MadeDecStageBwdArgs a, const MadeDecFold f) {
+    constexpr bool FOLD = HD > 0;
+    constexpr int DS_HD = FOLD ? HD : DS_BN, DS_FT = DS_HD / DS_BN, DS_FCT_LD = DS_HD + 4, DS_Q2_LD = DS_HD + 8, NC = FOLD ? HD / 16 : 1;
     constexpr bool TWO = MODE == 2, ADD1 = MODE == 1;
     constexpr int K = 64 * NV;
     constexpr int LDA = K * 2 + 16;
     constexpr int STEPS = NV / 2;
+    constexpr int FT = FOLD ? DS_FT : 1;
     __shared__ __attribute__((aligned(16))) unsigned char dlds[DS_BM * LDA];
-    __shared__ __attribute__((aligned(16))) float Ct[4 * DS_BM * DS_CT_LD];
+    __shared__ __attribute__((aligned(16))) float Ct[4 * DS_BM * (FOLD ? DS_FCT_LD : DS_CT_LD)];
+    __shared__ __attribute__((aligned(16))) bf16_t q2[FOLD ? DS_BM * DS_Q2_LD : 8];
     __shared__ float pgrad[4 * (TWO ? 4 : 2) * K];
     constexpr int PV = TWO ? 4 : 2;
     const int tid = threadIdx.x;
     const int lane = tid & 63, wave = __builtin_amdgcn_readfirstlane(tid >> 6);
     const int r16 = lane & 15, kq = lane >> 4;
     const int M = (int)a.M, N = (int)a.N;
-    const int n0 = blockIdx.x * DS_BN, m0 = blockIdx.y * DS_BM;
+    const int heads = FOLD ? N / DS_HD : 1;
+    const int fh = FOLD ? (int)blockIdx.x % heads : 0, fslice = FOLD ? (int)blockIdx.x / heads : 0;
+    const int n0 = FOLD ? fh * DS_HD : blockIdx.x * DS_BN, m0 = blockIdx.y * DS_BM;
     constexpr bool two = TWO;
+    const int r32 = lane & 31, hh = lane >> 5;
+    const int n2 = fslice * DS_SL + wave * 32 + r32;
+    bf16x8 fw2[NC];
+    if constexpr (FOLD) ds_fold_load<NC>(f.W2, f.ldw2, f.w2_z_stride, fh, n2, hh, fw2);
 
     const int kw = wave * (K / 4) + kq * 8;
-    int gn = n0 + r16; gn = gn < N ? gn : N - 1;
-    const bf16_t* pw = (const bf16_t*)a.W + (int64_t)gn * a.ldw + kw;
-    bf16x8 fw[STEPS];
-#pragma unroll
-    for (int s = 0; s < STEPS; ++s) fw[s] = *(const bf16x8*)(pw + s * 32);
-    const int cc = tid & 1, row = (tid >> 1) & 15;
+    bf16x8 fw[FT][STEPS];
+#pragma unroll
+    for (int t = 0; t < FT; ++t) {
+        int gn = n0 + t * DS_BN + r16; gn = gn < N ? gn : N - 1;
+        const bf16_t* pw = (const bf16_t*)a.W + (int64_t)gn * a.ldw + kw;
+#pragma unroll
+        for (int s = 0; s < STEPS; ++s) fw[t][s] = *(const bf16x8*)(pw + s * 32);
+    }
+    const int cc = FOLD ? (tid & (DS_HD / 8 - 1)) : (tid & 1), row = FOLD ? ((tid / (DS_HD / 8)) & 15) : ((tid >> 1) & 15);
     const int n = n0 + cc * 8;
     int nvalid = N - n; nvalid = nvalid > 8 ? 8 : nvalid;
     const int ml = m0 + row;
@@ -445,17 +536,22 @@
     }
     __syncthreads();
 
-    f32x4 acc;
-    acc[0] = acc[1] = acc[2] = acc[3] = 0.f;
+    f32x4 acc[FT];
+#pragma unroll
+    for (int t = 0; t < FT; ++t) acc[t][0] = acc[t][1] = acc[t][2] = acc[t][3] = 0.f;
 #pragma unroll
     for (int s = 0; s < STEPS; ++s) {
         const bf16x8 fa = *(const bf16x8*)(dlds + r16 * LDA + (kw + s * 32) * 2);
-        acc = __builtin_amdgcn_mfma_f32_16x16x32_bf16(fa, fw[s], acc, 0, 0, 0);
+#pragma unroll
+        for (int t = 0; t < FT; ++t) acc[t] = __builtin_amdgcn_mfma_f32_16x16x32_bf16(fa, fw[t][s], acc[t], 0, 0, 0);
     }
     {
-        float* mine = Ct + wave * (DS_BM * DS_CT_LD);
-#pragma unroll
-        for (int e = 0; e < 4; ++e) mine[(kq * 4 + e) * DS_CT_LD + r16] = acc[e];
+        constexpr int CT_LD = FOLD ? DS_FCT_LD : DS_CT_LD;
+        float* mine = Ct + wave * (DS_BM * CT_LD);
+#pragma unroll
+        for (int t = 0; t < FT; ++t)
+#pragma unroll
+            for (int e = 0; e < 4; ++e) mine[(kq * 4 + e) * CT_LD + t * DS_BN + r16] = acc[t][e];
     }
     if (blockIdx.x == 0) {
         for (int c = tid; c < PV * K; c += DS_THREADS) {
@@ -467,6 +563,28 @@
         }
     }
     __syncthreads();
+    if constexpr (FOLD) {
+        if (tid < 2 * DS_HD) {
+            float v8[8];
+#pragma unroll
+            for (int j = 0; j < 8; ++j) v8[j] = 0.f;
+#pragma unroll
+            for (int w = 0; w < 4; ++w) {
+                const float* cp = Ct + w * (DS_BM * DS_FCT_LD) + row * DS_FCT_LD + cc * 8;
+                const f32x4 q0 = *(const f32x4*)cp, q1 = *(const f32x4*)(cp + 4);
+                v8[0] += q0[0]; v8[1] += q0[1]; v8[2] += q0[2]; v8[3] += q0[3];
+                v8[4] += q1[0]; v8[5] += q1[1]; v8[6] += q1[2]; v8[7] += q1[3];
+            }
+            bf16x8 o;
+#pragma unroll
+            for (int j = 0; j < 8; ++j) o[j] = (bf16_t)v8[j];
+            *(bf16x8*)(q2 + row * DS_Q2_LD + cc * 8) = o;
+            if (fslice == 0 && ml < M) *(bf16x8*)((bf16_t*)a.out + (int64_t)ml * a.ldo + n) = o;
+        }
+        __syncthreads();
+        ds_fold_product<NC>(q2, fw2, f.out2, f.ldo2, f.out2_z_stride, fh, n2, r32, hh, m0, M);
+        return;
+    }
     if (tid >= 32 || nvalid <= 0 || ml >= M) return;
 
     float v8[8];
@@ -521,7 +639,17 @@
 
 }
 
-extern "C" int made_dec_stage_bwd(const MadeDecStageBwdArgs* args, void* stream) {
+static int ds_fold_check(const char* who, const MadeDecFold& f, int64_t N, const void* out, int64_t ldo) {
+    MADE_REQUIRE(f.W2 && f.out2, "%s: null W2 or out2", who);
+    MADE_UNSUPPORTED(f.hd == 64 || f.hd == 32, "%s: hd=%lld (the head width) must be 64 or 32", who, (long long)f.hd);
+    MADE_UNSUPPORTED(N > 0 && N % f.hd == 0, "%s: N=%lld must be heads * hd", who, (long long)N);
+    MADE_UNSUPPORTED(f.N2 > 0 && f.N2 % DS_SL == 0, "%s: N2=%lld must be a multiple of 128", who, (long long)f.N2);
+    MADE_UNSUPPORTED(f.ldw2 % 8 == 0 && f.w2_z_stride % 8 == 0 && ((uintptr_t)f.W2 % 16) == 0, "%s: W2 rows must be 16-byte aligned", who);
+    MADE_UNSUPPORTED(ldo % 8 == 0 && ((uintptr_t)out % 16) == 0, "%s: out rows must be 16-byte aligned", who);
+    return 0;
+}
+
+static int dec_stage_bwd_launch(const MadeDecStageBwdArgs* args, const MadeDecFold* fold, void* stream) {
     MADE_REQUIRE(args != nullptr, "made_dec_stage_bwd: null args");
     const MadeDecStageBwdArgs& a = *args;
     MADE_REQUIRE(a.xa && a.gamma_a && a.dy && a.W && a.out, "made_dec_stage_bwd: null xa, gamma_a, dy, W or out");
@@ -533,21 +661,41 @@
                      ((uintptr_t)a.dx_out % 16) == 0 && ((uintptr_t)a.a_out % 16) == 0 && ((uintptr_t)a.W % 16) == 0,
                      "made_dec_stage_bwd: rows must be 16-byte aligned");
     MADE_REQUIRE(a.drop_a.p >= 0.f && a.drop_a.p < 1.f && a.drop_o.p >= 0.f && a.drop_o.p < 1.f, "made_dec_stage_bwd: dropout p out of [0,1)");
-    const dim3 grid((unsigned)((a.N + DS_BN - 1) / DS_BN), (unsigned)((a.M + DS_BM - 1) / DS_BM)), block(DS_THREADS);
+    const dim3 block(DS_THREADS);
     hipStream_t st = (hipStream_t)stream;
+    if (fold) {
+        const MadeDecFold& f = *fold;
+        MADE_REQUIRE(a.xb == nullptr && a.add == nullptr && a.G == nullptr && a.R == nullptr && a.drop_o.p == 0.f,
+                     "made_dec_stage_bwd_fold: one norm, no add, gate, output dropout or residual");
+        if (const int rc = ds_fold_check("made_dec_stage_bwd_fold", f, a.N, a.out, a.ldo)) return rc;
+        const dim3 grid((unsigned)((f.N2 / DS_SL) * (a.N / f.hd)), (unsigned)((a.M + DS_BM - 1) / DS_BM));
+        if (a.K == 512 && f.hd == 64) hipLaunchKernelGGL((dec_stage_bwd_kernel<8, 0, 64>), grid, block, 0, st, a, f);
+        else if (a.K == 512) hipLaunchKernelGGL((dec_stage_bwd_kernel<8, 0, 32>), grid, block, 0, st, a, f);
+        else if (f.hd == 64) hipLaunchKernelGGL((dec_stage_bwd_kernel<4, 0, 64>), grid, block, 0, st, a, f);
+        else hipLaunchKernelGGL((dec_stage_bwd_kernel<4, 0, 32>), grid, block, 0, st, a, f);
+        return made_check_launch("made_dec_stage_bwd_fold");
+    }
+    const MadeDecFold f = {};
+    const dim3 grid((unsigned)((a.N + DS_BN - 1) / DS_BN), (unsigned)((a.M + DS_BM - 1) / DS_BM));
     if (a.K == 512) {
-        if (a.xb) hipLaunchKernelGGL((dec_stage_bwd_kernel<8, 2>), grid, block, 0, st, a);
-        else if (a.add) hipLaunchKernelGGL((dec_stage_bwd_kernel<8, 1>), grid, block, 0, st, a);
-        else hipLaunchKernelGGL((dec_stage_bwd_kernel<8, 0>), grid, block, 0, st, a);
+        if (a.xb) hipLaunchKernelGGL((dec_stage_bwd_kernel<8, 2>), grid, block, 0, st, a, f);
+        else if (a.add) hipLaunchKernelGGL((dec_stage_bwd_kernel<8, 1>), grid, block, 0, st, a, f);
+        else hipLaunchKernelGGL((dec_stage_bwd_kernel<8, 0>), grid, block, 0, st, a, f);
     } else {
-        if (a.xb) hipLaunchKernelGGL((dec_stage_bwd_kernel<4, 2>), grid, block, 0, st, a);
-        else if (a.add) hipLaunchKernelGGL((dec_stage_bwd_kernel<4, 1>), grid, block, 0, st, a);
-        else hipLaunchKernelGGL((dec_stage_bwd_kernel<4, 0>), grid, block, 0, st, a);
+        if (a.xb) hipLaunchKernelGGL((dec_stage_bwd_kernel<4, 2>), grid, block, 0, st, a, f);
+        else if (a.add) hipLaunchKernelGGL((dec_stage_bwd_kernel<4, 1>), grid, block, 0, st, a, f);
+        else hipLaunchKernelGGL((dec_stage_bwd_kernel<4, 0>), grid, block, 0, st, a, f);
     }
     return made_check_launch("made_dec_stage_bwd");
 }
 
-extern "C" int made_dec_stage(const MadeDecStageArgs* args, void* stream) {
+extern "C" int made_dec_stage_bwd(const MadeDecStageBwdArgs* args, void* stream) { return dec_stage_bwd_launch(args, nullptr, stream); }
+extern "C" int made_dec_stage_bwd_fold(const MadeDecStageBwdArgs* args, const MadeDecFold* fold, void* stream) {
+    MADE_REQUIRE(fold != nullptr, "made_dec_stage_bwd_fold: null fold");
+    return dec_stage_bwd_launch(args, fold, stream);
+}
+
+static int dec_stage_launch(const MadeDecStageArgs* args, const MadeDecFold* fold, void* stream) {
     MADE_REQUIRE(args != nullptr, "made_dec_stage: null args");
     const MadeDecStageArgs& a = *args;
     MADE_REQUIRE(a.Zin && a.W && a.out, "made_dec_stage: null Zin, W or out");
@@ -569,14 +717,33 @@
     if (a.zin_dtype == MADE_BF16) MADE_UNSUPPORTED(a.ldz % 8 == 0, "made_dec_stage: bf16 Zin rows must be 16-byte aligned");
     MADE_UNSUPPORTED((a.zin_dtype == MADE_BF16) == train || !train, "made_dec_stage: dropout / a_out need bf16 Zin rows");
     const bool tr = a.zin_dtype == MADE_BF16;
-    const dim3 grid((unsigned)((a.N + DS_BN - 1) / DS_BN), (unsigned)((a.M + DS_BM - 1) / DS_BM)), block(DS_THREADS);
+    const dim3 block(DS_THREADS);
     hipStream_t st = (hipStream_t)stream;
+    if (fold) {
+        const MadeDecFold& f = *fold;
+        MADE_REQUIRE(tr && a.out_dtype == MADE_BF16 && a.R == nullptr && !a.res_from_x, "made_dec_stage_fold: bf16 Zin and out, no residual");
+        if (const int rc = ds_fold_check("made_dec_stage_fold", f, a.N, a.out, a.ldo)) return rc;
+        const dim3 grid((unsigned)((f.N2 / DS_SL) * (a.N / f.hd)), (unsigned)((a.M + DS_BM - 1) / DS_BM));
+        if (a.K == 512 && f.hd == 64) hipLaunchKernelGGL((dec_stage_kernel<8, true, true, 64>), grid, block, 0, st, a, f);
+        else if (a.K == 512) hipLaunchKernelGGL((dec_stage_kernel<8, true, true, 32>), grid, block, 0, st, a, f);
+        else if (f.hd == 64) hipLaunchKernelGGL((dec_stage_kernel<4, true, true, 64>), grid, block, 0, st, a, f);
+        else hipLaunchKernelGGL((dec_stage_kernel<4, true, true, 32>), grid, block, 0, st, a, f);
+        return made_check_launch("made_dec_stage_fold");
+    }
+    const MadeDecFold f = {};
+    const dim3 grid((unsigned)((a.N + DS_BN - 1) / DS_BN), (unsigned)((a.M + DS_BM - 1) / DS_BM));
     if (a.K == 512) {
-        if (tr) hipLaunchKernelGGL((dec_stage_kernel<8, true, true>), grid, block, 0, st, a);
-        else hipLaunchKernelGGL((dec_stage_kernel<8, false, false>), grid, block, 0, st, a);
+        if (tr) hipLaunchKernelGGL((dec_stage_kernel<8, true, true>), grid, block, 0, st, a, f);
+        else hipLaunchKernelGGL((dec_stage_kernel<8, false, false>), grid, block, 0, st, a, f);
     } else {
-        if (tr) hipLaunchKernelGGL((dec_stage_kernel<4, true, true>), grid, block, 0, st, a);
-        else hipLaunchKernelGGL((dec_stage_kernel<4, false, false>), grid, block, 0, st, a);
+        if (tr) hipLaunchKernelGGL((dec_stage_kernel<4, true, true>), grid, block, 0, st, a, f);
+        else hipLaunchKernelGGL((dec_stage_kernel<4, false, false>), grid, block, 0, st, a, f);
     }
     return made_check_launch("made_dec_stage");
 }
+
+extern "C" int made_dec_stage(const MadeDecStageArgs* args, void* stream) { return dec_stage_launch(args, nullptr, stream); }
+extern "C" int made_dec_stage_fold(const MadeDecStageArgs* args, const MadeDecFold* fold, void* stream) {
+    MADE_REQUIRE(fold != nullptr, "made_dec_stage_fold: null fold");
+    return dec_stage_launch(args, fold, stream);
+}
diff --git a/mgsv_amd/ops.py b/mgsv_amd/ops.py
--- a/mgsv_amd/ops.py
+++ b/mgsv_amd/ops.py
@@ -9,7 +9,7 @@
 
 from . import _lib, tape as _tape
 from ._lib import (ACT_GELU, ACT_NONE, ACT_QUICKGELU, ACT_RELU, ACT_SIGMOID, BF16, F32,
-                   MadeAttnArgs, MadeDecStageArgs, MadeFinishArgs, MadeLinearArgs, MadeLinearSeg, MadeWideAttnArgs, check, lib)
+                   MadeAttnArgs, MadeDecFold, MadeDecStageArgs, MadeFinishArgs, MadeLinearArgs, MadeLinearSeg, MadeWideAttnArgs, check, lib)
 
 Tensor = torch.Tensor
 
@@ -297,7 +297,7 @@
 def dec_stage(Zin: Tensor, W: Tensor, bias: Optional[Tensor], out: Tensor, *, ln=None, ln2=None, x2_out: Optional[Tensor] = None,
               add: Optional[Tensor] = None, x_out: Optional[Tensor] = None, R: Optional[Tensor] = None, res_from_x: bool = False,
               act: int = ACT_NONE, eps: float = 1e-5, a_out: Optional[Tensor] = None, drop=None, drop_ld: Optional[int] = None,
-              drop_col_div: int = 1) -> Tensor:
+              drop_col_div: int = 1, fold_w: Optional[Tensor] = None, fold_w_z_stride: int = 0, fold_out: Optional[Tensor] = None) -> Tensor:
     assert Zin.dim() == 2 and W.dim() == 2 and out.dim() == 2 and W.dtype == torch.bfloat16
     assert Zin.stride(1) == 1 and W.stride(1) == 1 and out.stride(1) == 1
     M, K = Zin.shape
@@ -331,9 +331,25 @@
     a.out, a.ldo, a.out_dtype = _p(out), out.stride(0), dt_of(out)
     a.act, a.res_from_x, a.eps = act, 1 if res_from_x else 0, eps
     a.M, a.N, a.K = M, N, K
+    if fold_w is not None:
+        f = dec_fold_args(fold_w, fold_w_z_stride, fold_out, M, N)
+        _timed("dec_stage_fold_kernel", 2.0 * M * N * (K + f.N2), float(M * K * 2 * ((N + 31) // 32) + N * K * 2 + N * f.N2 * 2 + M * (N + N // f.hd * f.N2) * 2),
+               lambda: check(lib().made_dec_stage_fold(C.byref(a), C.byref(f), _stream()), "made_dec_stage_fold"), f"M={M} N={N} K={K} N2={f.N2}")
+        return out
     _timed("dec_stage_kernel", 2.0 * M * N * K, float(M * K * Zin.element_size() * ((N + 31) // 32) + N * K * 2 + M * N * out.element_size()),
            lambda: check(lib().made_dec_stage(C.byref(a), _stream()), "made_dec_stage"), f"M={M} N={N} K={K}")
     return out
+
+
+def dec_fold_args(fold_w: Tensor, fold_w_z_stride: int, fold_out: Tensor, M: int, N: int) -> MadeDecFold:
+    assert fold_w.dim() == 2 and fold_w.dtype == torch.bfloat16 and fold_w.stride(1) == 1
+    N2, hd = fold_w.shape
+    assert hd in (32, 64) and N % hd == 0 and N2 % 128 == 0
+    assert fold_out is not None and fold_out.dtype == torch.bfloat16 and tuple(fold_out.shape) == (M, N // hd, N2) and fold_out.stride(2) == 1
+    f = MadeDecFold()
+    f.W2, f.ldw2, f.w2_z_stride, f.N2 = _p(fold_w), fold_w.stride(0), int(fold_w_z_stride), N2
+    f.out2, f.ldo2, f.out2_z_stride, f.hd = _p(fold_out), fold_out.stride(0), fold_out.stride(1), hd
+    return f
 
 
 def attention(Q: Tensor, K: Tensor, V: Tensor, O: Tensor, H: int, *, key_mask: Optional[Tensor] = None,
diff --git a/mgsv_amd/ops_train.py b/mgsv_amd/ops_train.py
--- a/mgsv_amd/ops_train.py
+++ b/mgsv_amd/ops_train.py
@@ -7,7 +7,7 @@
 
 from . import _lib, tape as _tape
 from ._lib import BF16, F32, MadeAttnBwdArgs, MadeDropout, MadeGemmTNArgs, MadeGemmTNGroup, check, lib
-from .ops import _f32, _p, _stream, _timed, dt_of, set_drop
+from .ops import _f32, _p, _stream, _timed, dec_fold_args, dt_of, set_drop
 
 Tensor = torch.Tensor
 Pair = Tuple[int, int]
@@ -209,7 +209,8 @@
                   xb: Optional[Tensor] = None, gamma_b: Optional[Tensor] = None, dgamma_b: Optional[Tensor] = None, dbeta_b: Optional[Tensor] = None,
                   add: Optional[Tensor] = None, dx_out: Optional[Tensor] = None, a_out: Optional[Tensor] = None, drop_a=None,
                   G: Optional[Tensor] = None, gate_scale: float = 1.0, drop_o=None, drop_o_ld: int = 0, drop_o_col_div: int = 1,
-                  R: Optional[Tensor] = None, eps: float = 1e-5) -> Tensor:
+                  R: Optional[Tensor] = None, eps: float = 1e-5, fold_w: Optional[Tensor] = None, fold_w_z_stride: int = 0,
+                  fold_out: Optional[Tensor] = None) -> Tensor:
     from . import _lib as L
     M, K = xa.shape
     N = W.shape[0]
@@ -243,6 +244,11 @@
         a.R, a.ldr = _p(R), R.stride(0)
     a.out, a.ldo = _p(out), out.stride(0)
     a.M, a.N, a.K = M, N, K
+    if fold_w is not None:
+        f = dec_fold_args(fold_w, fold_w_z_stride, fold_out, M, N)
+        _timed("dec_stage_bwd_fold_kernel", 2.0 * M * N * (K + f.N2), float(M * K * 2 * 2 * ((N + 31) // 32) + N * K * 2 + N * f.N2 * 2 + M * (N + N // f.hd * f.N2) * 2),
+               lambda: check(lib().made_dec_stage_bwd_fold(C.byref(a), C.byref(f), _stream()), "made_dec_stage_bwd_fold"), f"M={M} N={N} K={K} N2={f.N2}")
+        return out
     _timed("dec_stage_bwd_kernel", 2.0 * M * N * K, float(M * K * 2 * 2 * ((N + 31) // 32) + N * K * 2 + M * N * 2),
            lambda: check(lib().made_dec_stage_bwd(C.byref(a), _stream()), "made_dec_stage_bwd"), f"M={M} N={N} K={K}")
     return out
diff --git a/mgsv_amd/trainer.py b/mgsv_amd/trainer.py
--- a/mgsv_amd/trainer.py
+++ b/mgsv_amd/trainer.py
@@ -761,6 +761,11 @@
         else:
             self._dec_self_attn_fwd(tw, l, tgt)
         ta = ops.linear(tw[d + ".att"], P[p + ".sa.out.w"], P[p + ".sa.out.b"], R=tgt, out=tw[d + ".t_a"], drop=self._drop(f"dec.{l}" + ".drop1", pd))
+        qprime = tw["GQ"][:, 1, l]
+        if stage and self._dec_fold(l):
+            ops.dec_stage(ta, Win[:D], bin_[:D], tw[d + ".qc"], ln=(P[p + ".ln1.g"], P[p + ".ln1.b"]), add=qp,
+                          x_out=tw[d + ".t1"], a_out=tw[d + ".t1q"], fold_w=Wt[:, D:D + hd], fold_w_z_stride=hd, fold_out=qprime)
+            return
         if stage:
             qc = ops.dec_stage(ta, Win[:D], bin_[:D], tw[d + ".qc"], ln=(P[p + ".ln1.g"], P[p + ".ln1.b"]), add=qp,
                                x_out=tw[d + ".t1"], a_out=tw[d + ".t1q"])
@@ -768,7 +773,6 @@
             ln = ".ln2" if pre else ".ln1"
             ops.layernorm_add(ta, P[p + ln + ".g"], P[p + ln + ".b"], qp_rows if pre else self._query_pos_rows(), tw[d + ".t1"], tw[d + ".t1q"])
             qc = ops.linear(tw[d + ".t1q"], Win[:D], bin_[:D], out=tw[d + ".qc"])
-        qprime = tw["GQ"][:, 1, l]
         ops.linear(qc[:, :hd], Wt[:, D:D + hd], None, M=B * Q, N=D, K=hd, batch=H, a_z_stride=hd, w_z_stride=hd,
                    segs=[Seg(out=qprime, ldo=D, rows_per_batch=Q, out_batch_stride=qprime.stride(0), out_z_stride=Q * D)])
 
@@ -914,6 +918,17 @@
         return (self.tc == torch.bfloat16 and c.num_moment_queries == 1 and c.D in (256, 512) and not c.detr_pre_norm
                 and _lib.variant_env("MADE_DEC_STAGE", "1") != "0")
 
+    DEC_FOLD_LAYERS = 3
+
+    def _dec_fold(self, l: int, backward: bool = False) -> bool:
+        c = self.cfg
+        if not (c.D // c.detr_nheads in (32, 64) and c.D % c.detr_nheads == 0):
+            return False
+        mode = _lib.variant_env("MADE_DEC_FOLD", "1")
+        if mode == "2":
+            return True
+        return mode != "0" and not backward and l >= max(1, c.detr_dec_layers - self.DEC_FOLD_LAYERS)
+
     def _encode_train(self, feats: Tensor, mask: Tensor, which: str, ws, tw, row_off: int) -> None:
         c, P = self.cfg, self.P
         if c.agg_module == "mlp":
@@ -1301,8 +1316,9 @@
             if pre:
                 pass
             elif stage:
+                fold = dict(fold_w=Wt[:, 2 * D:2 * D + hd], fold_w_z_stride=hd, fold_out=GQ[:, 0, l]) if self._dec_fold(l, backward=True) else {}
                 dattc = tr.dec_stage_bwd(tw[d + ".t_b"], P[p + ".ln2.g"], dt2, P[p + ".ca.out.wt"], g_attc, dgamma_a=G[p + ".ln2.g"],
-                                         dbeta_a=G[p + ".ln2.b"], dx_out=g2b, a_out=g_ca, drop_a=self._drop(f"dec.{l}" + ".drop2", pd))
+                                         dbeta_a=G[p + ".ln2.b"], dx_out=g2b, a_out=g_ca, drop_a=self._drop(f"dec.{l}" + ".drop2", pd), **fold)
             else:
                 tr.layernorm_bwd(tw[d + ".t_b"], P[p + ".ln2.g"], dt2, g2, dgamma=G[p + ".ln2.g"], dbeta=G[p + ".ln2.b"],
                                  dx_drop=g_ca, drop=self._drop(f"dec.{l}" + ".drop2", pd))
@@ -1310,8 +1326,9 @@
             dpooled = GQ[:, 0, l]
             qprime = GQ[:, 1, l]
             if stage:
-                ops.linear(dattc[:, :hd], Wt[:, 2 * D:2 * D + hd], None, M=B * Q, N=D, K=hd, batch=H, a_z_stride=hd, w_z_stride=hd,
-                           segs=[Seg(out=dpooled, ldo=D, rows_per_batch=Q, out_batch_stride=dpooled.stride(0), out_z_stride=Q * D)])
+                if not self._dec_fold(l, backward=True):
+                    ops.linear(dattc[:, :hd], Wt[:, 2 * D:2 * D + hd], None, M=B * Q, N=D, K=hd, batch=H, a_z_stride=hd, w_z_stride=hd,
+                               segs=[Seg(out=dpooled, ldo=D, rows_per_batch=Q, out_batch_stride=dpooled.stride(0), out_z_stride=Q * D)])
                 tr.attention_wide_bwd(qprime, dpooled, tw[d + ".pooled"].view(B, HQ, D), mempos3, mem3, tw["ca_lse"][l].view(B, HQ),
                                       PdS[:, 0, l], PdS[:, 1, l], g_q, scale=ca_scale, key_mask=fus_mask, ssum=tw[d + ".s"].view(B, HQ),
                                       dattc=dattc, vbias=P[p + ".ca.in.b"][2 * D:], hd=hd, drop=self._drop(f"dec.{l}" + ".ca_attn", pd),
```

New measurement: 14260 pairs/s, median of 6. No clear change (+0.2%).
